# Lymphatus/caesium-clt

Hardware: NVIDIA H100
Metric: megapixels/sec JPEG q=80 4K re-encode (higher is better)
Workload: dtype i32

## Files before the change

caesium-clt_b200/csrc/jpeg_gpuenc.cu:

```cuda
#include <cuda_runtime.h>
#include <cub/device/device_scan.cuh>
#include <cuda_pipeline.h>
#include <algorithm>
#include <chrono>
#include <cstring>
#include "jpeg_gpuenc.h"
#include "stream_wait.h"
#include "launch_timer.h"

namespace b200 {

using namespace ge;

__global__ void k_ge_groups(const Scan *__restrict__ scans, const uint32_t *__restrict__ meta, const int *__restrict__ evkey,
                            const int *__restrict__ prev, const uint32_t *__restrict__ tsum, uint32_t *__restrict__ gcount, uint32_t *__restrict__ hist)
{
    __shared__ uint32_t eob[16];
    const Scan s = scans[blockIdx.y];
    if (s.mode != MODE_AC_FIRST && s.mode != MODE_AC_REFINE) return;
    if ((int)(blockIdx.x * blockDim.x) > s.nblocks) return;
    if (threadIdx.x < 16) eob[threadIdx.x] = 0;
    __syncthreads();
    const int b = blockIdx.x * blockDim.x + threadIdx.x;
    if (b <= s.nblocks && (b == s.nblocks || meta_event(meta[s.unit_base + b]))) {
        int pg;
        if (b < s.nblocks) pg = prev[s.unit_base + b];
        else { const long long last = s.unit_base + s.nblocks - 1; pg = max(prev[last], evkey[last]); }
        const int pl = pg >= s.unit_base ? (int)(pg - s.unit_base) : -1;
        assign_groups(meta + s.unit_base, tsum + s.unit_base, s.nblocks, pl, b, gcount + s.unit_base,
                      [&](uint32_t c) { atomicAdd(&eob[eob_symbol(c) >> 4], 1u); });
    }
    __syncthreads();
    if (threadIdx.x < 16 && eob[threadIdx.x]) atomicAdd(&hist[((size_t)s.tab_base + 2 + s.tbl[0]) * 256 + (threadIdx.x << 4)], eob[threadIdx.x]);
}

__global__ void k_ge_tables(const uint32_t *__restrict__ hist, Table *__restrict__ tabs, DhtOut *__restrict__ dht)
{
    __shared__ long long freq[257];
    __shared__ int codesize[257], others[257];
    __shared__ uint8_t bits[33];
    const int t = blockIdx.x, lane = threadIdx.x;
    const uint32_t *f = hist + (size_t)t * 256;
    for (int i = lane; i < 257; i += 32) { freq[i] = i < 256 ? (long long)f[i] : 1; codesize[i] = 0; others[i] = -1; }
    if (lane == 0) for (int i = 0; i < 33; i++) bits[i] = 0;
    __syncwarp();
    auto warp_argmin = [&](int exclude) {
        unsigned long long v = 1000000000ULL; int c = -1;
        for (int i = lane; i < 257; i += 32) { const unsigned long long fi = (unsigned long long)freq[i]; if (fi && fi <= v && i != exclude) { v = fi; c = i; } }
        const unsigned hi = (unsigned)(v >> 32), lo = (unsigned)v;
        const unsigned mhi = __reduce_min_sync(0xFFFFFFFFu, hi);
        const unsigned mlo = __reduce_min_sync(0xFFFFFFFFu, hi == mhi ? lo : 0xFFFFFFFFu);
        return __reduce_max_sync(0xFFFFFFFFu, (hi == mhi && lo == mlo) ? c : -1);
    };
    for (;;) {
        const int c1 = warp_argmin(-1);
        const int c2 = c1 < 0 ? -1 : warp_argmin(c1);
        if (c2 < 0) break;
        if (lane == 0) {
            int a = c1, b = c2;
            freq[a] += freq[b]; freq[b] = 0;
            codesize[a]++; while (others[a] >= 0) { a = others[a]; codesize[a]++; }
            others[a] = b;
            codesize[b]++; while (others[b] >= 0) { b = others[b]; codesize[b]++; }
        }
        __syncwarp();
    }
    if (lane == 0) {
        Table &T = tabs[t];
        for (int i = 0; i <= 256; i++) if (codesize[i]) bits[codesize[i] > 32 ? 32 : codesize[i]]++;
        for (int i = 32; i > 16; i--) while (bits[i] > 0) {
            int j = i - 2; while (bits[j] == 0) j--;
            bits[i] -= 2; bits[i - 1]++; bits[j + 1] += 2; bits[j]--;
        }
        int i = 16; while (i > 0 && bits[i] == 0) i--;
        if (i > 0) bits[i]--;
        int start[34];
        for (int l = 0; l < 34; l++) start[l] = 0;
        for (int s = 0; s <= 255; s++) if (codesize[s]) start[min(codesize[s], 32) + 1]++;
        for (int l = 1; l < 34; l++) start[l] += start[l - 1];
        const int p = start[33];
        for (int s = 0; s <= 255; s++) if (codesize[s]) T.vals[start[min(codesize[s], 32)]++] = (uint8_t)s;
        T.nvals = p;
        for (int k = 0; k < 17; k++) T.bits[k] = bits[k];
        for (int s = 0; s < 256; s++) T.code_len[s] = 0;
        uint32_t code = 0; int k = 0;
        for (int l = 1; l <= 16; l++) { for (int n = 0; n < bits[l]; n++, k++) T.code_len[T.vals[k]] = (code++ << 8) | (uint32_t)l; code <<= 1; }
        DhtOut &D = dht[t];
        D.nvals = p;
        for (int k2 = 0; k2 < 17; k2++) D.bits[k2] = bits[k2];
        for (int k2 = 0; k2 < p; k2++) D.vals[k2] = T.vals[k2];
    }
}

__global__ void k_ge_scanout(const Scan *__restrict__ scans, int nscans, const uint32_t *__restrict__ bitlen, const uint32_t *__restrict__ bitoff, uint32_t *__restrict__ total,
                             ScanOut *__restrict__ so, uint32_t words_cap, uint32_t groups_cap, uint32_t *__restrict__ flags)
{
    const int lane = threadIdx.x;
    uint32_t wbase = 0, gbase = 0;
    for (int c0 = 0; c0 < nscans; c0 += 32) {
        const int i = c0 + lane;
        uint32_t tb = 0;
        if (i < nscans) { const Scan s = scans[i]; const long long last = s.unit_base + s.nblocks - 1; tb = s.nblocks ? bitoff[last] + bitlen[last] - bitoff[s.unit_base] : 0; }
        const uint32_t nbytes = (tb + 7) / 8, ng = (nbytes + 15) / 16, nw = i < nscans ? (tb + 31) / 32 + 1 : 0;
        uint32_t wi = nw, gi = i < nscans ? ng : 0;
        for (int d = 1; d < 32; d <<= 1) { const uint32_t a = __shfl_up_sync(0xFFFFFFFFu, wi, d), b = __shfl_up_sync(0xFFFFFFFFu, gi, d); if (lane >= d) { wi += a; gi += b; } }
        if (i < nscans) { total[i] = tb; ScanOut o; o.total_bits = tb; o.nbytes = nbytes; o.ngroups = ng; o.group_base = gbase + gi - ng; o.word_base = wbase + wi - nw; o.pad_ = 0; so[i] = o; }
        wbase += __shfl_sync(0xFFFFFFFFu, wi, 31); gbase += __shfl_sync(0xFFFFFFFFu, gi, 31);
    }
    __syncwarp();
    const bool ovf = wbase > words_cap || gbase > groups_cap;
    if (lane == 0) { flags[0] = ovf ? 1u : 0u; flags[1] = wbase; flags[2] = gbase; flags[3] = 0; flags[4] = 0; }
    if (ovf) for (int i = lane; i < nscans; i += 32) { so[i].total_bits = 0; so[i].nbytes = 0; so[i].ngroups = 0; so[i].group_base = 0; so[i].word_base = 0; }
}

__global__ void k_ge_zero(const ScanOut *__restrict__ so, uint32_t *__restrict__ words)
{
    const ScanOut o = so[blockIdx.y];
    if (!o.total_bits) return;
    const uint32_t n = (o.total_bits + 31) / 32 + 1;
    uint32_t *w = words + o.word_base;
    for (uint32_t i = blockIdx.x * blockDim.x + threadIdx.x; i < n; i += gridDim.x * blockDim.x) w[i] = 0;
}

constexpr int ENC_THREADS = 128;
constexpr int TILE_PITCH = 72;
typedef int16_t Tile[ENC_THREADS][TILE_PITCH];

__device__ __forceinline__ void stage_tile(Tile &tile, const BlockComp &bc, int i0, int nblk)
{
    const uint4 *src = reinterpret_cast<const uint4 *>(bc.coef + bc.comp_off + (long long)i0 * 64);
    const int n = min(ENC_THREADS, nblk - i0) * 8;
#pragma unroll
    for (int k = 0; k < 8; k++) { const int q = threadIdx.x + k * ENC_THREADS; if (q < n) __pipeline_memcpy_async(&tile[q >> 3][(q & 7) * 8], src + q, 16); }
    __pipeline_commit();
}
__device__ __forceinline__ void wait_tile()
{
    __pipeline_wait_prior(0);
    __syncthreads();
}

__device__ __forceinline__ void stage_visits(EncVisit *vis, const BlockComp &bc)
{
    if ((int)threadIdx.x < bc.nscan) vis[threadIdx.x] = bc.visit[threadIdx.x];
}
__device__ __forceinline__ BlockRef ref_of(const EncVisit &v, const BlockComp &bc, const Tile &tile, int i0, int row, int col)
{
    BlockRef r;
    r.blk = tile[threadIdx.x]; r.prev = nullptr; r.slot = 0;
    if (v.mode == MODE_SEQ || v.mode == MODE_DC_FIRST) {
        const int p = enc_dc_prev(bc, v.ns, row, col);
        if (p >= i0 && p < i0 + ENC_THREADS) r.prev = tile[p - i0];
        else if (p >= 0) r.prev = bc.coef + bc.comp_off + (long long)p * 64;
    }
    return r;
}

template <class T>
__device__ __forceinline__ KindTabs<T> kind_tabs(T *tab, const EncVisit &v) { return KindTabs<T>{tab + ENC_DC_ENTRY, tab + v.ac_entry}; }

__device__ __forceinline__ Masks3 load_masks(const Masks3 *__restrict__ masks, const BlockComp &bc, int i)
{
    const unsigned long long *q = reinterpret_cast<const unsigned long long *>(masks + bc.mask_base + i);
    Masks3 M;
    M.m[0] = __ldg(q); M.m[1] = __ldg(q + 1); M.m[2] = __ldg(q + 2);
    return M;
}

struct SmemHist {
    KindTabs<uint32_t> h;
    __device__ void sym(int kind, int, int symbol, int, unsigned) { atomicAdd((kind ? h.ac : h.dc) + symbol, 1u); }
    __device__ void raw64(int, unsigned long long) {}
};
__global__ void __launch_bounds__(ENC_THREADS) k_geb_classify(const BlockComp *__restrict__ comps, uint32_t *__restrict__ meta, int *__restrict__ evkey,
                                                              uint32_t *__restrict__ tail, Masks3 *__restrict__ masks, uint32_t *__restrict__ hist)
{
    __shared__ __align__(16) Tile tile;
    __shared__ uint32_t h[ENC_TAB_ENTRIES];
    __shared__ EncVisit vis[ENC_MAX_VISITS];
    const BlockComp &bc = comps[blockIdx.y];
    const int nblk = bc.bw * bc.bh, i0 = blockIdx.x * ENC_THREADS, i = i0 + threadIdx.x;
    if (i0 >= nblk) return;
    stage_tile(tile, bc, i0, nblk);
    for (int k = threadIdx.x; k < ENC_TAB_ENTRIES; k += ENC_THREADS) h[k] = 0;
    stage_visits(vis, bc);
    wait_tile();
    if (i < nblk) {
        const int row = i / bc.bw, col = i - row * bc.bw;
        const Masks3 M = make_masks3(tile[threadIdx.x]);
        masks[bc.mask_base + i] = M;
        for (int j = 0; j < bc.nscan; j++) {
            const EncVisit &v = vis[j];
            const int u = enc_unit_of(bc, v.ns, row, col);
            if (u < 0) continue;
            const uint32_t m = classify_m(v, M);
            const int g = v.unit_base + u;
            meta[g] = m; evkey[g] = meta_event(m) ? g : -1; tail[g] = (uint32_t)meta_tail(m);
            SmemHist sk{kind_tabs(h, v)};
            gen_block_m(v, v.tbl, ref_of(v, bc, tile, i0, row, col), M, 0, sk);
        }
    }
    __syncthreads();
    for (int k = threadIdx.x; k < ENC_TAB_ENTRIES; k += ENC_THREADS) {
        int symbol; const int t = enc_entry_table(bc, k, symbol);
        if (h[k]) atomicAdd(&hist[(size_t)t * 256 + symbol], h[k]);
    }
}

__global__ void __launch_bounds__(ENC_THREADS) k_geb_len(const BlockComp *__restrict__ comps, const uint32_t *__restrict__ gcount, const Table *__restrict__ tabs,
                                                         uint32_t *__restrict__ bitlen, const Masks3 *__restrict__ masks)
{
    __shared__ __align__(16) Tile tile;
    __shared__ uint8_t tl[ENC_TAB_ENTRIES];
    __shared__ EncVisit vis[ENC_MAX_VISITS];
    const BlockComp &bc = comps[blockIdx.y];
    const int nblk = bc.bw * bc.bh, i0 = blockIdx.x * ENC_THREADS, i = i0 + threadIdx.x;
    if (i0 >= nblk) return;
    stage_tile(tile, bc, i0, nblk);
    const Masks3 M = load_masks(masks, bc, min(i, nblk - 1));
    stage_visits(vis, bc);
    for (int k = threadIdx.x; k < ENC_TAB_ENTRIES; k += ENC_THREADS) {
        int symbol; const int t = enc_entry_table(bc, k, symbol);
        if (t >= 0) tl[k] = (uint8_t)tabs[t].code_len[symbol];
    }
    wait_tile();
    if (i >= nblk) return;
    const int row = i / bc.bw, col = i - row * bc.bw;
    for (int j = 0; j < bc.nscan; j++) {
        const EncVisit &v = vis[j];
        const int u = enc_unit_of(bc, v.ns, row, col);
        if (u < 0) continue;
        LenSinkT<KindTabs<const uint8_t>> sk{kind_tabs<const uint8_t>(tl, v)};
        gen_block_m(v, v.tbl, ref_of(v, bc, tile, i0, row, col), M, gcount[v.unit_base + u], sk);
        bitlen[v.unit_base + u] = (uint32_t)sk.bits;
    }
}

__global__ void __launch_bounds__(ENC_THREADS) k_geb_emit(const BlockComp *__restrict__ comps, const uint32_t *__restrict__ gcount, const Table *__restrict__ tabs,
                                                          const uint32_t *__restrict__ bitoff, uint32_t *__restrict__ words, const Masks3 *__restrict__ masks, const ScanOut *__restrict__ so,
                                                          const uint32_t *__restrict__ flags)
{
    __shared__ __align__(16) Tile tile;
    __shared__ uint32_t tc[ENC_TAB_ENTRIES];
    __shared__ EncVisit vis[ENC_MAX_VISITS];
    __shared__ uint32_t vword[ENC_MAX_VISITS], vbit0[ENC_MAX_VISITS];
    if (flags[0]) return;
    const BlockComp &bc = comps[blockIdx.y];
    const int nblk = bc.bw * bc.bh, i0 = blockIdx.x * ENC_THREADS, i = i0 + threadIdx.x;
    if (i0 >= nblk) return;
    stage_tile(tile, bc, i0, nblk);
    const Masks3 M = load_masks(masks, bc, min(i, nblk - 1));
    stage_visits(vis, bc);
    if ((int)threadIdx.x < bc.nscan) {
        const EncVisit &v = bc.visit[threadIdx.x];
        vword[threadIdx.x] = so[v.scan].word_base; vbit0[threadIdx.x] = bitoff[v.unit_base];
    }
    for (int k = threadIdx.x; k < ENC_TAB_ENTRIES; k += ENC_THREADS) {
        int symbol; const int t = enc_entry_table(bc, k, symbol);
        if (t >= 0) tc[k] = tabs[t].code_len[symbol];
    }
    wait_tile();
    if (i >= nblk) return;
    const int row = i / bc.bw, col = i - row * bc.bw;
    auto orw = [&](long long w, uint32_t v) { if (v) atomicOr(&words[w], v); };
    auto stw = [&](long long w, uint32_t v) { words[w] = v; };
    for (int j = 0; j < bc.nscan; j++) {
        const EncVisit &v = vis[j];
        const int u = enc_unit_of(bc, v.ns, row, col);
        if (u < 0) continue;
        EmitSink<decltype(orw), decltype(stw), KindTabs<const uint32_t>> sk(kind_tabs<const uint32_t>(tc, v), orw, stw, (long long)vword[j],
                                                                            (unsigned long long)(bitoff[v.unit_base + u] - vbit0[j]));
        gen_block_m(v, v.tbl, ref_of(v, bc, tile, i0, row, col), M, gcount[v.unit_base + u], sk);
        sk.finish();
    }
}

__device__ __forceinline__ uint32_t scan_byte(const uint32_t *__restrict__ w, uint32_t i, uint32_t nbytes, uint32_t total_bits)
{
    uint32_t b = (w[i >> 2] >> (24 - 8 * (i & 3))) & 0xFF;
    if (i == nbytes - 1 && (total_bits & 7)) b |= (1u << (8 - (total_bits & 7))) - 1u;
    return b;
}

__global__ void k_ge_ffcount(const ScanOut *__restrict__ so, int nscans, const uint32_t *__restrict__ words, uint32_t *__restrict__ ffcount, uint32_t groups_cap,
                             const uint32_t *__restrict__ flags)
{
    if ((int)blockIdx.y == nscans) {
        const uint32_t used = flags[0] ? 0u : flags[2];
        for (uint32_t g = used + blockIdx.x * blockDim.x + threadIdx.x; g < groups_cap; g += gridDim.x * blockDim.x) ffcount[g] = 0;
        return;
    }
    const ScanOut o = so[blockIdx.y];
    const uint32_t *w = words + o.word_base;
    for (uint32_t g = blockIdx.x * blockDim.x + threadIdx.x; g < o.ngroups; g += gridDim.x * blockDim.x) {
        uint32_t n = 0;
        for (uint32_t i = g * 16; i < g * 16 + 16 && i < o.nbytes; i++) n += scan_byte(w, i, o.nbytes, o.total_bits) == 0xFF;
        ffcount[o.group_base + g] = n;
    }
}

__global__ void k_ge_layout(const ScanOut *__restrict__ so, int scans_per_image, int nimages, const uint32_t *__restrict__ ffcount, const uint32_t *__restrict__ ffoff,
                            uint32_t *__restrict__ out_off, uint32_t *__restrict__ out_len, uint32_t out_image_stride, uint32_t *__restrict__ flags)
{
    const int im = blockIdx.x * blockDim.x + threadIdx.x;
    if (im >= nimages) return;
    uint32_t off = 0;
    for (int k = 0; k < scans_per_image; k++) {
        const int si = im * scans_per_image + k;
        const ScanOut o = so[si];
        uint32_t ff = 0;
        if (o.ngroups) { const uint32_t lastg = o.group_base + o.ngroups - 1; ff = ffoff[lastg] + ffcount[lastg] - ffoff[o.group_base]; }
        out_off[si] = off; out_len[si] = o.nbytes + ff;
        off += o.nbytes + ff;
    }
    atomicMax(&flags[3], off);
    if (off > out_image_stride) atomicOr(&flags[4], 1u);
}

__global__ void k_ge_scatter(const ScanOut *__restrict__ so, const uint32_t *__restrict__ words, const uint32_t *__restrict__ ffoff,
                             const uint32_t *__restrict__ out_off, uint8_t *__restrict__ out, int scans_per_image, size_t out_image_stride, const uint32_t *__restrict__ flags)
{
    if (flags[4]) return;
    const ScanOut o = so[blockIdx.y];
    const uint32_t *w = words + o.word_base;
    uint8_t *base = out + (size_t)(blockIdx.y / scans_per_image) * out_image_stride + out_off[blockIdx.y];
    for (uint32_t g = blockIdx.x * blockDim.x + threadIdx.x; g < o.ngroups; g += gridDim.x * blockDim.x) {
        uint8_t *dst = base + (size_t)g * 16 + (ffoff[o.group_base + g] - ffoff[o.group_base]);
        for (uint32_t i = g * 16; i < g * 16 + 16 && i < o.nbytes; i++) {
            const uint32_t b = scan_byte(w, i, o.nbytes, o.total_bits);
            *dst++ = (uint8_t)b;
            if (b == 0xFF) *dst++ = 0;
        }
    }
}

__global__ void k_ge_fill_dummy(int16_t *__restrict__ coef, long long comp_off, int bw, int bh, int rbw, int rbh, int hs)
{
    const int i = blockIdx.x * blockDim.x + threadIdx.x;
    if (i >= bw * bh) return;
    const int row = i / bw, col = i - row * bw;
    if (row < rbh && col < rbw) return;
    int r = row, c = col;
    while (r >= rbh || c >= rbw) { if (r >= rbh) { c = (c / hs) * hs + hs - 1; r--; } else c = rbw - 1; }
    int16_t *base = coef + comp_off;
    int16_t *dst = base + ((long long)row * bw + col) * 64;
    const int16_t dc = base[((long long)r * bw + c) * 64];
    for (int k = 1; k < 64; k++) dst[k] = 0;
    dst[0] = dc;
}

static inline size_t align_up(size_t v, size_t a) { return (v + a - 1) / a * a; }
static inline int cdiv(long long a, long long b) { return (int)((a + b - 1) / b); }

GpuEncoder::~GpuEncoder()
{
    if (ev_sizes) cudaEventDestroy((cudaEvent_t)ev_sizes);
}

bool GpuEncoder::size_back_buffers(size_t image_bytes, std::string &err)
{
    const int NS = (int)plan.scans.size();
    if (nimg != cap_nimg) { cap_nimg = nimg; est_image_bytes = 0; }
    if (image_bytes <= est_image_bytes && words_cap) return true;
    est_image_bytes = image_bytes + image_bytes / 8;
    image_bytes = est_image_bytes;
    words_cap = (uint32_t)std::min<size_t>((size_t)nimg * (image_bytes / 4 + 1) + 2 * (size_t)NS + 64, 0xFFFFFF00u);
    groups_cap = (uint32_t)((size_t)words_cap / 4 + NS + 1);
    out_stride = align_up(image_bytes + image_bytes / 8 + 1024, 256);
    auto grow = [&](auto &buf, size_t need) { return buf.reserve(need, Grow::Pow2Half, err, &generation); };
    if (!grow(d_words, (size_t)words_cap * 4 + 64) || !grow(d_ffcount, (size_t)groups_cap * 4 + 4) || !grow(d_ffoff, (size_t)groups_cap * 4 + 4) ||
        !grow(d_out, out_stride * nimg)) return false;
    size_t tb3 = 0; cub::DeviceScan::ExclusiveSum((void *)nullptr, tb3, d_ffcount.get(), d_ffoff.get(), (int)groups_cap, (cudaStream_t)0);
    return grow(d_temp, tb3 + 256);
}

bool GpuEncoder::prepare(const JpegGeom &g, bool progressive, int16_t *const *d_coefs, int nimages, void *stream_, size_t out_bytes_hint, std::string &err)
{
    cudaStream_t st = (cudaStream_t)stream_;
    geom = g; prog = progressive;
    std::vector<const int16_t *> bases(d_coefs, d_coefs + nimages);
    coef_bases.assign(d_coefs, d_coefs + nimages);
    gpuenc_plan(g, progressive, bases.data(), nimages, plan);
    nimg = nimages;
    const int NS = (int)plan.scans.size();
    const long long U = plan.total_units;
    if (U >= (1ll << 31)) { err = "batch too large for the entropy encoder"; return false; }
    overflow = false;
    for (auto &sc_ : plan.scans) if (!masks_cover(sc_.mode, sc_.Al)) { err = "scan script outside the device encoder's mask range"; overflow = true; return false; }
    if (!plan.on_chip) { err = "scan script outside the device encoder's on-chip table slots"; overflow = true; return false; }
    if (!ev_sizes) { cudaEvent_t e; CU(cudaEventCreateWithFlags(&e, cudaEventDisableTiming | (stream_wait_mode() == 0 ? 0 : cudaEventBlockingSync))); ev_sizes = e; }
    auto grow = [&](auto &buf, size_t need) { return buf.reserve(need, Grow::Pow2Half, err, &generation); };
    const int NC = (int)plan.comps.size();
    if (!grow(d_scans, NS * sizeof(Scan)) || !grow(d_comps, NC * sizeof(BlockComp)) ||
        !grow(d_meta, U * 4) || !grow(d_evkey, U * 4) || !grow(d_prev, U * 4) || !grow(d_tail, U * 4) || !grow(d_tsum, U * 4) ||
        !grow(d_gcount, U * 4) || !grow(d_bitlen, U * 4) || !grow(d_bitoff, U * 4) ||
        !grow(d_hist, (size_t)NS * 4 * 256 * 4) || !grow(d_tabs, (size_t)NS * 4 * sizeof(Table)) || !grow(d_dht, (size_t)NS * 4 * sizeof(DhtOut)) ||
        !grow(d_total, (size_t)NS * 4) || !grow(d_so, (size_t)NS * sizeof(ScanOut)) || !grow(d_outoff, (size_t)NS * 4) || !grow(d_outlen, (size_t)NS * 4) ||
        !grow(d_flags, 64) || !grow(d_masks, (size_t)plan.total_comp_blocks * sizeof(Masks3))) return false;
    o_scans = 0; o_total = o_scans + align_up((size_t)NS * sizeof(Scan), 256); o_outlen = o_total + align_up((size_t)NS * 4, 256);
    o_dht = o_outlen + align_up((size_t)NS * 4, 256); o_comps = o_dht + align_up((size_t)NS * 4 * sizeof(DhtOut), 256);
    o_flags = o_comps + align_up((size_t)NC * sizeof(BlockComp), 256);
    const size_t small_bytes = o_flags + 256;
    if (!grow(h_small, small_bytes)) return false;
    size_t tb1 = 0, tb2 = 0;
    cub::DeviceScan::ExclusiveScan((void *)nullptr, tb1, d_evkey.get(), d_prev.get(), cub::Max(), -1, (int)U, st);
    cub::DeviceScan::ExclusiveSum((void *)nullptr, tb2, d_tail.get(), d_tsum.get(), (int)U, st);
    if (!grow(d_temp, std::max(tb1, tb2) + 256)) return false;
    const size_t coef_bytes = (size_t)g.total_coefs * 2;
    if (coef_bytes != learned_for) { learned_for = coef_bytes; learned_image_bytes = 0; }
    size_t est = out_bytes_hint ? out_bytes_hint / nimages + out_bytes_hint / nimages / 4 : coef_bytes / 3;
    est = std::max(est, learned_image_bytes + learned_image_bytes / 8) + 8192;
    est = std::min(est, coef_bytes * 2 + (size_t)plan.scans_per_image * 64 + 8192);
    if (!size_back_buffers(est, err)) return false;
    memcpy(h_small + o_scans, plan.scans.data(), NS * sizeof(Scan));
    memcpy(h_small + o_comps, plan.comps.data(), NC * sizeof(BlockComp));
    (void)st;
    return true;
}

bool GpuEncoder::upload(void *stream_, std::string &err)
{
    cudaStream_t st = (cudaStream_t)stream_;
    const int NS = (int)plan.scans.size(), NC = (int)plan.comps.size();
    CU(cudaMemcpyAsync(d_scans, h_small + o_scans, NS * sizeof(Scan), cudaMemcpyHostToDevice, st));
    CU(cudaMemcpyAsync(d_comps, h_small + o_comps, NC * sizeof(BlockComp), cudaMemcpyHostToDevice, st));
    return true;
}

unsigned long long GpuEncoder::signature() const
{
    unsigned long long h = 1469598103934665603ull;
    auto mix = [&](unsigned long long v) { h = (h ^ v) * 1099511628211ull; };
    mix((unsigned long long)nimg); mix((unsigned long long)plan.scans.size()); mix((unsigned long long)plan.comps.size()); mix((unsigned long long)plan.total_units);
    mix((unsigned long long)plan.max_comp_blocks); mix((unsigned long long)plan.scans_per_image); mix(words_cap); mix(groups_cap); mix(out_stride); mix(generation);
    mix((unsigned long long)geom.width); mix((unsigned long long)geom.height); mix(prog ? 1 : 0);
    for (int c = 0; c < geom.ncomp; c++) { mix((unsigned long long)geom.bw[c]); mix((unsigned long long)geom.bh[c]); mix((unsigned long long)geom.rbw[c]); mix((unsigned long long)geom.rbh[c]); mix((unsigned long long)geom.hs[c]); }
    for (auto pb : coef_bases) mix((unsigned long long)(uintptr_t)pb);
    int max_units = 0; for (auto &sc : plan.scans) max_units = std::max(max_units, sc.nblocks);
    mix((unsigned long long)max_units);
    return h;
}

bool GpuEncoder::enqueue_sizes(void *stream_, std::string &err)
{
    cudaStream_t st = (cudaStream_t)stream_;
    const int NS = (int)plan.scans.size();
    uint32_t *h_total = reinterpret_cast<uint32_t *>(h_small + o_total), *h_flags = reinterpret_cast<uint32_t *>(h_small + o_flags);
    k_ge_scanout<<<1, 32, 0, st>>>(d_scans, NS, d_bitlen, d_bitoff, d_total, d_so, words_cap, groups_cap, d_flags);
    LT_MARK("k_ge_scanout");
    CU(cudaMemcpyAsync(h_total, d_total, (size_t)NS * 4, cudaMemcpyDeviceToHost, st));
    CU(cudaMemcpyAsync(h_flags, d_flags, 12, cudaMemcpyDeviceToHost, st));
    LT_MARK("copy");
    return true;
}
bool GpuEncoder::mark_sizes(void *stream_, std::string &err)
{
    CU(cudaEventRecord((cudaEvent_t)ev_sizes, (cudaStream_t)stream_));
    return true;
}

bool GpuEncoder::enqueue_back(void *stream_, std::string &err)
{
    cudaStream_t st = (cudaStream_t)stream_;
    const int NS = (int)plan.scans.size(), NC = (int)plan.comps.size();
    uint32_t *h_flags = reinterpret_cast<uint32_t *>(h_small + o_flags);
    const dim3 gb(cdiv(plan.max_comp_blocks, ENC_THREADS), NC);
    k_ge_zero<<<dim3(64, NS), 256, 0, st>>>(d_so, d_words);
    LT_MARK("k_ge_zero");
    k_geb_emit<<<gb, ENC_THREADS, 0, st>>>(d_comps, d_gcount, d_tabs, d_bitoff, d_words, d_masks, d_so, d_flags);
    LT_MARK("k_geb_emit");
    k_ge_ffcount<<<dim3(32, NS + 1), 128, 0, st>>>(d_so, NS, d_words, d_ffcount, groups_cap, d_flags);
    LT_MARK("k_ge_ffcount");
    size_t tb = d_temp.capacity();
    cub::DeviceScan::ExclusiveSum(d_temp, tb, d_ffcount.get(), d_ffoff.get(), (int)groups_cap, st);
    LT_MARK("cub_scan");
    k_ge_layout<<<cdiv(nimg, 64), 64, 0, st>>>(d_so, plan.scans_per_image, nimg, d_ffcount, d_ffoff, d_outoff, d_outlen, (uint32_t)out_stride, d_flags);
    LT_MARK("k_ge_layout");
    k_ge_scatter<<<dim3(32, NS), 128, 0, st>>>(d_so, d_words, d_ffoff, d_outoff, d_out, plan.scans_per_image, out_stride, d_flags);
    LT_MARK("k_ge_scatter");
    CU(cudaMemcpyAsync(h_small + o_outlen, d_outlen, (size_t)NS * 4, cudaMemcpyDeviceToHost, st));
    CU(cudaMemcpyAsync(h_small + o_dht, d_dht, (size_t)NS * 4 * sizeof(DhtOut), cudaMemcpyDeviceToHost, st));
    CU(cudaMemcpyAsync(h_flags + 4, d_flags, 32, cudaMemcpyDeviceToHost, st));
    CU(cudaGetLastError());
    launches += 7;
    return true;
}

bool GpuEncoder::enqueue(void *stream_, bool fill_dummy, std::string &err)
{
    return enqueue_front(stream_, fill_dummy, err) && enqueue_sizes(stream_, err) && mark_sizes(stream_, err) && enqueue_back(stream_, err);
}

bool GpuEncoder::enqueue_front(void *stream_, bool fill_dummy, std::string &err)
{
    cudaStream_t st = (cudaStream_t)stream_;
    const JpegGeom &g = geom;
    const int NS = (int)plan.scans.size(), NC = (int)plan.comps.size();
    const long long U = plan.total_units;
    int max_units = 0; for (auto &s : plan.scans) max_units = std::max(max_units, s.nblocks);
    launches = 0;
    const dim3 gb(cdiv(plan.max_comp_blocks, ENC_THREADS), NC);
    if (fill_dummy) {
        for (int im = 0; im < nimg; im++) for (int cc = 0; cc < g.ncomp; cc++) {
            if (g.rbw[cc] == g.bw[cc] && g.rbh[cc] == g.bh[cc]) continue;
            k_ge_fill_dummy<<<cdiv((long long)g.bw[cc] * g.bh[cc], 256), 256, 0, st>>>(coef_bases[im], g.comp_offset[cc], g.bw[cc], g.bh[cc], g.rbw[cc], g.rbh[cc], g.hs[cc]);
            LT_MARK("k_ge_fill_dummy");
            launches++;
        }
    }
    const dim3 gu1(cdiv(max_units + 1, 128), NS);
    CU(cudaMemsetAsync(d_hist, 0, (size_t)NS * 4 * 256 * 4, st));
    LT_MARK("memset");
    k_geb_classify<<<gb, ENC_THREADS, 0, st>>>(d_comps, d_meta, d_evkey, d_tail, d_masks, d_hist);
    LT_MARK("k_geb_classify");
    size_t tb = d_temp.capacity();
    cub::DeviceScan::ExclusiveScan(d_temp, tb, d_evkey.get(), d_prev.get(), cub::Max(), -1, (int)U, st);
    LT_MARK("cub_scan");
    tb = d_temp.capacity();
    cub::DeviceScan::ExclusiveSum(d_temp, tb, d_tail.get(), d_tsum.get(), (int)U, st);
    LT_MARK("cub_scan");
    CU(cudaMemsetAsync(d_gcount, 0, U * 4, st));
    LT_MARK("memset");
    k_ge_groups<<<gu1, 128, 0, st>>>(d_scans, d_meta, d_evkey, d_prev, d_tsum, d_gcount, d_hist);
    LT_MARK("k_ge_groups");
    k_ge_tables<<<NS * 4, 32, 0, st>>>(d_hist, d_tabs, d_dht);
    LT_MARK("k_ge_tables");
    k_geb_len<<<gb, ENC_THREADS, 0, st>>>(d_comps, d_gcount, d_tabs, d_bitlen, d_masks);
    LT_MARK("k_geb_len");
    tb = d_temp.capacity();
    cub::DeviceScan::ExclusiveSum(d_temp, tb, d_bitlen.get(), d_bitoff.get(), (int)U, st);
    LT_MARK("cub_scan");
    launches += 7;
    CU(cudaGetLastError());
    return true;
}

bool GpuEncoder::finish(void *stream_, bool fetch, std::string &err)
{
    cudaStream_t st = (cudaStream_t)stream_;
    const int NS = (int)plan.scans.size(), spi = plan.scans_per_image;
    uint32_t *h_total = reinterpret_cast<uint32_t *>(h_small + o_total), *h_flags = reinterpret_cast<uint32_t *>(h_small + o_flags);
    uint32_t *h_outlen = reinterpret_cast<uint32_t *>(h_small + o_outlen);
    const DhtOut *h_dht = reinterpret_cast<const DhtOut *>(h_small + o_dht);
    for (int attempt = 0;; attempt++) {
        const auto tw0 = std::chrono::steady_clock::now();
        if (fetch) { CU(event_wait((cudaEvent_t)ev_sizes)); } else { CU(stream_wait(st)); }
        wait_sizes_ms = std::chrono::duration<double, std::milli>(std::chrono::steady_clock::now() - tw0).count();
        size_t img_max = 0, img = 0;
        for (int si = 0; si < NS; si++) { img += (h_total[si] + 7) / 8; if ((si + 1) % spi == 0) { img_max = std::max(img_max, img); img = 0; } }
        if (h_flags[0]) {
            if (attempt >= 3) { err = "entropy encoder could not size its buffers"; return false; }
            CU(stream_wait(st));
            if (!size_back_buffers(img_max + img_max / 16 + 4096, err)) return false;
            retries++;
            if (!enqueue_sizes(st, err) || !mark_sizes(st, err) || !enqueue_back(st, err)) return false;
            continue;
        }
        if (fetch) {
            copy_bytes = std::min(out_stride, align_up(img_max + img_max / 8 + 256, 256));
            if (!h_out.reserve(copy_bytes * nimg, Grow::Pow2Half, err, &generation)) return false;
            for (int im = 0; im < nimg; im++) CU(cudaMemcpyAsync(h_out + (size_t)im * copy_bytes, d_out + (size_t)im * out_stride, copy_bytes, cudaMemcpyDeviceToHost, st));
            CU(cudaGetLastError());
            const auto tw1 = std::chrono::steady_clock::now();
            CU(stream_wait(st));
            wait_final_ms = std::chrono::duration<double, std::milli>(std::chrono::steady_clock::now() - tw1).count();
        }
        if (h_flags[4 + 4]) {
            if (attempt >= 3) { err = "entropy encoder could not size its output"; return false; }
            if (!size_back_buffers((size_t)h_flags[4 + 3] + 4096, err)) return false;
            retries++;
            if (!enqueue_sizes(st, err) || !mark_sizes(st, err) || !enqueue_back(st, err)) return false;
            continue;
        }
        learned_image_bytes = std::max<size_t>(learned_image_bytes, h_flags[4 + 3]);
        if (fetch) {
            bool shortc = false;
            for (int im = 0; im < nimg && !shortc; im++) { size_t tot = 0; for (int k = 0; k < spi; k++) tot += h_outlen[im * spi + k]; shortc = tot > copy_bytes; }
            if (shortc) {
                if (!h_out.reserve(out_stride * nimg, Grow::Pow2Half, err, &generation)) return false;
                copy_bytes = out_stride;
                for (int j = 0; j < nimg; j++) CU(cudaMemcpyAsync(h_out + (size_t)j * copy_bytes, d_out + (size_t)j * out_stride, copy_bytes, cudaMemcpyDeviceToHost, st));
                CU(stream_wait(st));
            }
        }
        break;
    }
    results.assign((size_t)NS, EncodedScan());
    for (int si = 0; si < NS; si++) {
        EncodedScan &e = results[si];
        const int im = si / spi, k = si % spi;
        e.def = plan.defs[k];
        size_t off = 0; for (int j = 0; j < k; j++) off += h_outlen[im * spi + j];
        e.data = fetch ? h_out + (size_t)im * copy_bytes + off : nullptr; e.len = h_outlen[si];
        bool need[2][2]; jpeg_scan_tables_needed(geom, prog, e.def, need);
        for (int kind = 0; kind < 2; kind++) for (int t = 0; t < 2; t++) {
            e.has_tab[kind][t] = need[kind][t];
            const DhtOut &D = h_dht[(size_t)si * 4 + kind * 2 + t];
            memcpy(e.bits[kind][t], D.bits, 17); memcpy(e.vals[kind][t], D.vals, 256); e.nvals[kind][t] = D.nvals;
        }
    }
    return true;
}

bool GpuEncoder::encode(const JpegGeom &g, bool progressive, int16_t *const *d_coefs, int nimages, void *stream_, bool fill_dummy, std::string &err, size_t out_bytes_hint)
{
    return prepare(g, progressive, d_coefs, nimages, stream_, out_bytes_hint, err) && upload(stream_, err) && enqueue(stream_, fill_dummy, err) && finish(stream_, true, err);
}

}
```

caesium-clt_b200/csrc/jpeg_gpuenc.h:

```cpp
#pragma once
#include <cstdint>
#include <cstddef>
#include <string>
#include <vector>
#include "dev_buffer.h"
#include "jpeg_gpuenc_plan.h"

namespace b200 {

struct DhtOut { uint8_t bits[17]; uint8_t vals[256]; int32_t nvals; };
struct ScanOut { uint32_t total_bits, nbytes, ngroups, group_base, word_base, pad_; };

class GpuEncoder {
public:
    GpuEncoder() = default;
    ~GpuEncoder();
    GpuEncoder(const GpuEncoder &) = delete;
    GpuEncoder &operator=(const GpuEncoder &) = delete;
    bool encode(const JpegGeom &g, bool progressive, int16_t *const *d_coefs, int nimages, void *stream, bool fill_dummy, std::string &err, size_t out_bytes_hint = 0);
    bool prepare(const JpegGeom &g, bool progressive, int16_t *const *d_coefs, int nimages, void *stream, size_t out_bytes_hint, std::string &err);
    bool upload(void *stream, std::string &err);
    bool enqueue(void *stream, bool fill_dummy, std::string &err);
    bool enqueue_front(void *stream, bool fill_dummy, std::string &err);
    bool enqueue_sizes(void *stream, std::string &err);
    bool mark_sizes(void *stream, std::string &err);
    bool enqueue_back(void *stream, std::string &err);
    unsigned long long signature() const;
    bool finish(void *stream, bool fetch, std::string &err);
    int retries = 0;
    double wait_sizes_ms = 0, wait_final_ms = 0;
    std::vector<EncodedScan> results;
    GpuEncPlan plan;
    bool overflow = false;
    int launches = 0;
private:
    bool size_back_buffers(size_t image_bytes, std::string &err);
    unsigned long long generation = 0;
    int cap_nimg = 0;
    int nimg = 0;
    JpegGeom geom; bool prog = false;
    std::vector<int16_t *> coef_bases;
    void *ev_sizes = nullptr;
    uint32_t words_cap = 0, groups_cap = 0;
    size_t est_image_bytes = 0, learned_image_bytes = 0, learned_for = 0;
    DeviceBuffer<uint32_t> d_flags;
    size_t o_scans = 0, o_total = 0, o_outlen = 0, o_dht = 0, o_comps = 0, o_flags = 0;
    DeviceBuffer<ge::Scan> d_scans;
    DeviceBuffer<BlockComp> d_comps;
    DeviceBuffer<uint32_t> d_meta, d_tail, d_tsum, d_gcount, d_bitlen, d_bitoff;
    DeviceBuffer<int> d_evkey, d_prev;
    DeviceBuffer<uint32_t> d_hist;
    DeviceBuffer<ge::Table> d_tabs;
    DeviceBuffer<DhtOut> d_dht;
    DeviceBuffer<uint32_t> d_total;
    DeviceBuffer<ScanOut> d_so;
    DeviceBuffer<uint32_t> d_words;
    DeviceBuffer<ge::Masks3> d_masks;
    DeviceBuffer<uint32_t> d_ffcount, d_ffoff;
    DeviceBuffer<uint32_t> d_outoff, d_outlen;
    DeviceBuffer<uint8_t> d_out;
    DeviceBuffer<uint8_t> d_temp;
    PinnedBuffer<uint8_t> h_small;
    PinnedBuffer<uint8_t> h_out;
    size_t out_stride = 0, copy_bytes = 0;
};

}
```

caesium-clt_b200/csrc/jpeg_gpuenc_core.h:

```cpp
#pragma once
#include <cstdint>

#if defined(__CUDACC__)
#define GE_HD __host__ __device__ __forceinline__
#else
#define GE_HD inline
#endif

namespace b200 {
namespace ge {

enum ScanMode { MODE_SEQ = 0, MODE_DC_FIRST = 1, MODE_AC_FIRST = 2, MODE_AC_REFINE = 3 };

constexpr int EOBRUN_MAX = 0x7FFF;
constexpr int CORR_FLUSH = 1000 - 64 + 1;

struct Scan {
    const int16_t *coef;
    int mode, ns, Ss, Se, Al;
    int comp[3];
    int hs[3], vs[3], bw[3];
    long long comp_off[3];
    int tbl[3];
    int mcux, mcuy, blocks_per_mcu;
    int rbw, rbh;
    int nblocks;
    long long unit_base;
    int tab_base;
    long long word_base;
    long long word_cap;
};

struct Table {
    uint32_t code_len[256];
    uint8_t bits[17];
    uint8_t vals[256];
    int nvals;
};

GE_HD uint32_t meta_pack(bool event, bool contrib, int tail) { return (event ? 1u : 0u) | (contrib ? 2u : 0u) | ((uint32_t)tail << 8); }
GE_HD bool meta_event(uint32_t m) { return m & 1u; }
GE_HD bool meta_contrib(uint32_t m) { return m & 2u; }
GE_HD int meta_tail(uint32_t m) { return (int)(m >> 8); }

GE_HD int nbits_of(unsigned v)
{
#if defined(__CUDA_ARCH__)
    return 32 - __clz((int)v);
#else
    return v ? 32 - __builtin_clz(v) : 0;
#endif
}

struct BlockRef { const int16_t *blk; const int16_t *prev; int slot; };

GE_HD BlockRef locate(const Scan &s, int u)
{
    BlockRef r;
    if (s.ns == 1) {
        const int row = u / s.rbw, col = u - row * s.rbw;
        const int16_t *base = s.coef + s.comp_off[0];
        r.blk = base + ((long long)row * s.bw[0] + col) * 64;
        r.slot = 0;
        if (u == 0) r.prev = nullptr;
        else { const int pu = u - 1, prow = pu / s.rbw, pcol = pu - prow * s.rbw; r.prev = base + ((long long)prow * s.bw[0] + pcol) * 64; }
        return r;
    }
    const int m = u / s.blocks_per_mcu;
    int q = u - m * s.blocks_per_mcu, i = 0;
    while (q >= s.hs[i] * s.vs[i]) { q -= s.hs[i] * s.vs[i]; i++; }
    const int my = m / s.mcux, mx = m - my * s.mcux;
    const int by = q / s.hs[i], bx = q - by * s.hs[i];
    const int16_t *base = s.coef + s.comp_off[i];
    r.slot = i;
    r.blk = base + ((long long)(my * s.vs[i] + by) * s.bw[i] + mx * s.hs[i] + bx) * 64;
    if (q > 0) { const int pq = q - 1, pby = pq / s.hs[i], pbx = pq - pby * s.hs[i]; r.prev = base + ((long long)(my * s.vs[i] + pby) * s.bw[i] + mx * s.hs[i] + pbx) * 64; }
    else if (m == 0) r.prev = nullptr;
    else { const int pm = m - 1, pmy = pm / s.mcux, pmx = pm - pmy * s.mcux; r.prev = base + ((long long)(pmy * s.vs[i] + s.vs[i] - 1) * s.bw[i] + pmx * s.hs[i] + s.hs[i] - 1) * 64; }
    return r;
}

GE_HD int ctz64(unsigned long long m)
{
#if defined(__CUDA_ARCH__)
    return __ffsll((long long)m) - 1;
#else
    return __builtin_ctzll(m);
#endif
}
GE_HD int msb64(unsigned long long m)
{
#if defined(__CUDA_ARCH__)
    return 63 - __clzll((long long)m);
#else
    return m ? 63 - __builtin_clzll(m) : -1;
#endif
}
GE_HD int popc64(unsigned long long m)
{
#if defined(__CUDA_ARCH__)
    return __popcll(m);
#else
    return __builtin_popcountll(m);
#endif
}
GE_HD unsigned long long band_mask(int Ss, int Se) { return (Se >= 63 ? ~0ull : ((1ull << (Se + 1)) - 1ull)) & ~((1ull << Ss) - 1ull); }

struct Masks3 { unsigned long long m[3]; };
GE_HD bool masks_cover(int mode, int Al) { return mode == MODE_AC_REFINE ? Al <= 1 : Al <= 2; }
GE_HD unsigned long long mask_at(const Masks3 &M, int t) { return t == 0 ? M.m[0] : t == 1 ? M.m[1] : M.m[2]; }

GE_HD uint32_t interleave16(uint32_t acc)
{
    uint32_t x = acc & 0xFFFFu, y = acc >> 16;
    x = (x | (x << 8)) & 0x00FF00FFu; x = (x | (x << 4)) & 0x0F0F0F0Fu; x = (x | (x << 2)) & 0x33333333u; x = (x | (x << 1)) & 0x55555555u;
    y = (y | (y << 8)) & 0x00FF00FFu; y = (y | (y << 4)) & 0x0F0F0F0Fu; y = (y | (y << 2)) & 0x33333333u; y = (y | (y << 1)) & 0x55555555u;
    return x | (y << 1);
}
GE_HD void masks_word(uint32_t w, int jj , uint32_t (&acc)[3])
{
    const uint32_t sb = (w >> 15) & 0x00010001u;
    const uint32_t a = (w ^ (sb * 0xFFFFu)) + sb;
    const uint32_t pos = 0x00010001u << jj;
    acc[0] |= ((a + 0x7FFF7FFFu) >> (15 - jj)) & pos;
    acc[1] |= (((a & 0xFFFEFFFEu) + 0x7FFF7FFFu) >> (15 - jj)) & pos;
    acc[2] |= (((a & 0xFFFCFFFCu) + 0x7FFF7FFFu) >> (15 - jj)) & pos;
}
GE_HD Masks3 make_masks3(const int16_t *__restrict__ blk)
{
    Masks3 M;
    uint32_t lo[3] = {0, 0, 0}, hi[3] = {0, 0, 0};
#if defined(__CUDA_ARCH__)
    const uint4 *v = reinterpret_cast<const uint4 *>(blk);
#pragma unroll
    for (int j = 0; j < 8; j++) {
        const uint4 q = v[j];
        const uint32_t w[4] = {q.x, q.y, q.z, q.w};
#pragma unroll
        for (int i = 0; i < 4; i++) { if (j < 4) masks_word(w[i], (4 * j + i) & 15, lo); else masks_word(w[i], (4 * j + i) & 15, hi); }
    }
#else
    for (int j = 0; j < 32; j++) {
        const uint32_t w = (uint32_t)(uint16_t)blk[2 * j] | ((uint32_t)(uint16_t)blk[2 * j + 1] << 16);
        if (j < 16) masks_word(w, j, lo); else masks_word(w, j - 16, hi);
    }
#endif
    for (int t = 0; t < 3; t++) M.m[t] = ((unsigned long long)interleave16(hi[t]) << 32) | interleave16(lo[t]);
    return M;
}
inline Masks3 make_masks3_reference(const int16_t *blk)
{
    Masks3 M; M.m[0] = M.m[1] = M.m[2] = 0;
    for (int k = 0; k < 64; k++) { int a = blk[k]; if (a < 0) a = -a; for (int t = 0; t < 3; t++) if (a >= (1 << t)) M.m[t] |= 1ull << k; }
    return M;
}

template <class S>
GE_HD uint32_t classify_m(const S &s, const Masks3 &M)
{
    if (s.mode == MODE_SEQ || s.mode == MODE_DC_FIRST) return meta_pack(true, false, 0);
    const unsigned long long band = band_mask(s.Ss, s.Se);
    const unsigned long long mA = mask_at(M, s.Al) & band, mB = (s.mode == MODE_AC_REFINE ? mask_at(M, s.Al + 1) : 0ull) & band;
    if (s.mode == MODE_AC_FIRST) { const int last = msb64(mA); return meta_pack(last >= 0, last < s.Se, 0); }
    const int last_new = msb64(mA & ~mB);
    int tail;
    if (last_new < 0) tail = popc64(mB);
    else if (last_new >= 63) tail = 0;
    else tail = popc64(mB & ~((2ull << last_new) - 1ull));
    return meta_pack(last_new >= 0, last_new < s.Se, tail);
}
GE_HD uint32_t classify(const Scan &s, const int16_t *blk)
{
    if (s.mode == MODE_SEQ || s.mode == MODE_DC_FIRST) return meta_pack(true, false, 0);
    return classify_m(s, make_masks3(blk));
}

template <class Sink>
GE_HD void gen_dc(int value_shifted, int pred_shifted, int tbl, Sink &sk)
{
    int temp = value_shifted - pred_shifted, temp2 = temp;
    if (temp < 0) { temp = -temp; temp2--; }
    const int nb = nbits_of((unsigned)temp);
    sk.sym(0, tbl, nb, nb, (unsigned)temp2);
}

GE_HD int eob_symbol(unsigned count) { return (nbits_of(count) - 1) << 4; }
template <class Sink>
GE_HD void gen_eob_token(unsigned count, int tbl, Sink &sk)
{
    sk.sym(1, tbl, eob_symbol(count), nbits_of(count) - 1, count);
}

template <class S, class Sink>
GE_HD void gen_block_m(const S &s, int tbl, const BlockRef &b, const Masks3 &M, unsigned group_count, Sink &sk)
{
    const int16_t *blk = b.blk;
    if (s.mode == MODE_DC_FIRST) { gen_dc(blk[0] >> s.Al, b.prev ? (b.prev[0] >> s.Al) : 0, tbl, sk); return; }
    if (s.mode == MODE_SEQ) {
        gen_dc(blk[0], b.prev ? b.prev[0] : 0, tbl, sk);
        int prevk = 0;
        for (unsigned long long m = M.m[0] & ~1ull; m; m &= m - 1) {
            const int k = ctz64(m);
            int r = k - prevk - 1; prevk = k;
            while (r > 15) { sk.sym(1, tbl, 0xF0, 0, 0); r -= 16; }
            int t = blk[k], t2 = t; if (t < 0) { t = -t; t2--; }
            const int nb = nbits_of((unsigned)t);
            sk.sym(1, tbl, (r << 4) + nb, nb, (unsigned)t2);
        }
        if (prevk != 63) sk.sym(1, tbl, 0, 0, 0);
        return;
    }
    const unsigned long long band = band_mask(s.Ss, s.Se);
    const unsigned long long mA = mask_at(M, s.Al) & band;
    const unsigned long long mB = (s.mode == MODE_AC_REFINE ? mask_at(M, s.Al + 1) : 0ull) & band;
    if (s.mode == MODE_AC_FIRST) {
        int prevk = s.Ss - 1;
        for (unsigned long long m = mA; m; m &= m - 1) {
            const int k = ctz64(m);
            int r = k - prevk - 1; prevk = k;
            while (r > 15) { sk.sym(1, tbl, 0xF0, 0, 0); r -= 16; }
            int t = blk[k], t2;
            if (t < 0) { t = (-t) >> s.Al; t2 = ~t; } else { t >>= s.Al; t2 = t; }
            const int nb = nbits_of((unsigned)t);
            sk.sym(1, tbl, (r << 4) + nb, nb, (unsigned)t2);
        }
        if (group_count) gen_eob_token(group_count, tbl, sk);
        return;
    }
    const unsigned long long newm = mA & ~mB;
    const int last_new = msb64(newm);
    const int EOB = last_new < 0 ? 0 : last_new;
    int r = 0, prevk = s.Ss - 1;
    int npend = 0; unsigned long long pend64 = 0;
    for (unsigned long long m = mA; m; m &= m - 1) {
        const int k = ctz64(m);
        r += k - prevk - 1; prevk = k;
        while (r > 15 && k <= EOB) {
            sk.sym(1, tbl, 0xF0, 0, 0); r -= 16;
            if (npend) { sk.raw64(npend, pend64); npend = 0; pend64 = 0; }
        }
        int t = blk[k];
        const bool neg = t < 0;
        if (neg) t = -t;
        t >>= s.Al;
        if ((mB >> k) & 1ull) { pend64 = (pend64 << 1) | (unsigned)(t & 1); npend++; continue; }
        sk.sym(1, tbl, (r << 4) + 1, 1, neg ? 0u : 1u);
        if (npend) { sk.raw64(npend, pend64); npend = 0; pend64 = 0; }
        r = 0;
    }
    if (group_count) gen_eob_token(group_count, tbl, sk);
    if (npend) sk.raw64(npend, pend64);
}
template <class Sink>
GE_HD void gen_block(const Scan &s, const BlockRef &b, unsigned group_count, Sink &sk)
{
    if (s.mode == MODE_DC_FIRST) { Masks3 none; none.m[0] = none.m[1] = none.m[2] = 0; gen_block_m(s, s.tbl[b.slot], b, none, group_count, sk); return; }
    gen_block_m(s, s.tbl[b.slot], b, make_masks3(b.blk), group_count, sk);
}

struct ScanTabs {
    const Table *t = nullptr;
    ScanTabs() = default;
    GE_HD ScanTabs(const Table *p) : t(p) {}
    GE_HD uint32_t operator()(int kind, int tbl, int symbol) const { return t[kind * 2 + tbl].code_len[symbol]; }
};
template <class T>
struct KindTabs {
    T *dc, *ac;
    GE_HD uint32_t operator()(int kind, int, int symbol) const { return (kind ? ac : dc)[symbol]; }
};

template <class AddFn>
struct HistSink {
    AddFn add;
    GE_HD explicit HistSink(AddFn f) : add(f) {}
    GE_HD void sym(int kind, int tbl, int symbol, int, unsigned) { add((kind * 2 + tbl) * 256 + symbol); }
    GE_HD void raw64(int, unsigned long long) {}
};

template <class Tabs = ScanTabs>
struct LenSinkT {
    Tabs tabs;
    unsigned long long bits = 0;
    GE_HD void sym(int kind, int tbl, int symbol, int nb, unsigned) { bits += (tabs(kind, tbl, symbol) & 0xFFu) + nb; }
    GE_HD void raw64(int nb, unsigned long long) { bits += nb; }
};
using LenSink = LenSinkT<>;

GE_HD uint32_t shl_or_zero(uint32_t v, int s)
{
#if defined(__CUDA_ARCH__)
    return __funnelshift_lc(0u, v, (unsigned)s);
#else
    return s >= 32 ? 0u : v << s;
#endif
}

template <class OrFn, class StFn = OrFn, class Tabs = ScanTabs>
struct EmitSink {
    Tabs tabs;
    OrFn orw;
    StFn stw;
    long long wpos, first;
    uint32_t cur = 0; int n;
    GE_HD EmitSink(Tabs t, OrFn f, StFn g, long long word_base, unsigned long long bitoff)
        : tabs(t), orw(f), stw(g), wpos(word_base + (long long)(bitoff >> 5)), first(wpos), n((int)(bitoff & 31)) {}
    GE_HD EmitSink(Tabs t, OrFn f, long long word_base, unsigned long long bitoff) : EmitSink(t, f, f, word_base, bitoff) {}
    GE_HD void put(uint32_t code, int len)
    {
        if (!len) return;
        const int fill = n + len;
        if (fill < 32) { cur |= code << (32 - fill); n = fill; return; }
        const int r = fill - 32;
        const uint32_t w = cur | (code >> r);
        if (wpos == first) orw(wpos, w); else stw(wpos, w);
        wpos++;
        cur = shl_or_zero(code, 32 - r); n = r;
    }
    GE_HD void sym(int kind, int tbl, int symbol, int nb, unsigned extra)
    {
        const uint32_t e = tabs(kind, tbl, symbol);
        put(((e >> 8) << nb) | (extra & ((1u << nb) - 1u)), (int)(e & 0xFFu) + nb);
    }
    GE_HD void raw64(int nb, unsigned long long v)
    {
        if (nb > 32) { put((unsigned)(v >> 32), nb - 32); put((unsigned)v, 32); } else put((unsigned)v, nb);
    }
    GE_HD void finish() { if (n > 0) orw(wpos, cur); }
};

struct NoCount { GE_HD void operator()(uint32_t) const {} };
template <class CountFn = NoCount>
GE_HD void assign_groups(const uint32_t *meta, const uint32_t *tsum, int nblocks, int prev_ev, int b, uint32_t *gcount, CountFn &&counted = CountFn())
{
    auto group = [&](int j, uint32_t c) { gcount[j] = c; counted(c); };
    int gs = prev_ev < 0 ? 0 : (meta_contrib(meta[prev_ev]) ? prev_ev : prev_ev + 1);
    if (gs >= b) return;
    const int count = b - gs;
    const uint32_t tend = b < nblocks ? tsum[b] : tsum[nblocks - 1] + (uint32_t)meta_tail(meta[nblocks - 1]);
    const uint32_t tailbits = tend - tsum[gs];
    if (count < EOBRUN_MAX && tailbits <= (uint32_t)CORR_FLUSH) { group(gs, (uint32_t)count); return; }
    int start = gs, n = 0; unsigned be = 0;
    for (int j = gs; j < b; j++) {
        n++; be += (unsigned)meta_tail(meta[j]);
        if (n == EOBRUN_MAX || be > (unsigned)CORR_FLUSH) { group(start, (uint32_t)n); start = j + 1; n = 0; be = 0; }
    }
    if (n > 0) group(start, (uint32_t)n);
}

GE_HD void build_table(const uint32_t *freq_in, Table &t, int *codesize , int *others , long long *freq )
{
    uint8_t bits[33];
    for (int i = 0; i < 33; i++) bits[i] = 0;
    for (int i = 0; i < 256; i++) { freq[i] = freq_in[i]; codesize[i] = 0; others[i] = -1; }
    freq[256] = 1; codesize[256] = 0; others[256] = -1;
    for (;;) {
        int c1 = -1, c2 = -1; long long v = 1000000000LL;
        for (int i = 0; i <= 256; i++) if (freq[i] && freq[i] <= v) { v = freq[i]; c1 = i; }
        v = 1000000000LL;
        for (int i = 0; i <= 256; i++) if (freq[i] && freq[i] <= v && i != c1) { v = freq[i]; c2 = i; }
        if (c2 < 0) break;
        freq[c1] += freq[c2]; freq[c2] = 0;
        codesize[c1]++; while (others[c1] >= 0) { c1 = others[c1]; codesize[c1]++; }
        others[c1] = c2;
        codesize[c2]++; while (others[c2] >= 0) { c2 = others[c2]; codesize[c2]++; }
    }
    for (int i = 0; i <= 256; i++) if (codesize[i]) bits[codesize[i] > 32 ? 32 : codesize[i]]++;
    for (int i = 32; i > 16; i--) while (bits[i] > 0) {
        int j = i - 2; while (bits[j] == 0) j--;
        bits[i] -= 2; bits[i - 1]++; bits[j + 1] += 2; bits[j]--;
    }
    int i = 16; while (i > 0 && bits[i] == 0) i--;
    if (i > 0) bits[i]--;
    for (int k = 0; k < 17; k++) t.bits[k] = bits[k];
    int p = 0;
    for (int l = 1; l <= 32; l++) for (int s = 0; s <= 255; s++) if (codesize[s] == l) t.vals[p++] = (uint8_t)s;
    t.nvals = p;
    for (int s = 0; s < 256; s++) t.code_len[s] = 0;
    uint32_t code = 0; int k = 0;
    for (int l = 1; l <= 16; l++) { for (int n = 0; n < t.bits[l]; n++, k++) t.code_len[t.vals[k]] = (code++ << 8) | (uint32_t)l; code <<= 1; }
}

}
}
```

caesium-clt_b200/csrc/jpeg_gpuenc_plan.h:

```cpp
#pragma once
#include <algorithm>
#include <vector>
#include "jpeg_gpuenc_core.h"
#include "jpeg_host.h"

namespace b200 {

constexpr int ENC_MAX_VISITS = 6, ENC_AC_SLOTS = 3, ENC_DC_SLOTS = 1, ENC_DC_SYMBOLS = 17;
constexpr int ENC_TAB_ENTRIES = ENC_AC_SLOTS * 256 + ENC_DC_SLOTS * ENC_DC_SYMBOLS;
constexpr int ENC_DC_ENTRY = ENC_AC_SLOTS * 256;

struct EncVisit {
    int scan;
    int mode, Ss, Se, Al, ns;
    int tbl;
    int unit_base;
    int ac_entry;
};

struct BlockComp {
    const int16_t *coef;
    long long comp_off;
    int bw, bh, rbw, rbh, hs, vs;
    int q_base, blocks_per_mcu, mcux;
    int nscan;
    EncVisit visit[ENC_MAX_VISITS];
    int tab[ENC_AC_SLOTS + ENC_DC_SLOTS];
    long long mask_base;
};

GE_HD int enc_unit_of(const BlockComp &bc, int ns, int row, int col)
{
    if (ns == 1) return (row < bc.rbh && col < bc.rbw) ? row * bc.rbw + col : -1;
    const int m = (row / bc.vs) * bc.mcux + col / bc.hs, q = bc.q_base + (row % bc.vs) * bc.hs + (col % bc.hs);
    return m * bc.blocks_per_mcu + q;
}
GE_HD int enc_dc_prev(const BlockComp &bc, int ns, int row, int col)
{
    if (ns == 1) return col > 0 ? row * bc.bw + col - 1 : row > 0 ? (row - 1) * bc.bw + bc.rbw - 1 : -1;
    if (col % bc.hs) return row * bc.bw + col - 1;
    if (row % bc.vs) return (row - 1) * bc.bw + col + bc.hs - 1;
    if (col) return (row + bc.vs - 1) * bc.bw + col - 1;
    if (row) return (row - 1) * bc.bw + bc.mcux * bc.hs - 1;
    return -1;
}

GE_HD int enc_entry_table(const BlockComp &bc, int k, int &symbol)
{
    if (k < ENC_DC_ENTRY) { symbol = k & 255; return bc.tab[k >> 8]; }
    symbol = k - ENC_DC_ENTRY; return bc.tab[ENC_AC_SLOTS];
}

struct GpuEncPlan {
    std::vector<BlockComp> comps;
    bool on_chip = true;
    int max_comp_blocks = 0;
    std::vector<ge::Scan> scans;
    std::vector<ScanDef> defs;
    int scans_per_image = 0;
    long long units_per_image = 0, words_per_image = 0;
    long long total_units = 0, total_words = 0, total_comp_blocks = 0;
};

inline void gpuenc_plan(const JpegGeom &g, bool progressive, const int16_t *const *coef_base, int nimages, GpuEncPlan &p)
{
    ScanDef sc[16];
    const int ns = jpeg_scan_script(g, progressive, sc);
    p.defs.assign(sc, sc + ns);
    p.scans_per_image = ns;
    p.scans.clear();
    long long unit = 0, word = 0;
    for (int im = 0; im < nimages; im++) {
        for (int si = 0; si < ns; si++) {
            const ScanDef &d = sc[si];
            ge::Scan s{};
            s.coef = coef_base[im];
            s.ns = d.ns; s.Ss = d.Ss; s.Se = d.Se; s.Al = d.Al;
            if (!progressive) s.mode = ge::MODE_SEQ;
            else if (d.Ss == 0) s.mode = ge::MODE_DC_FIRST;
            else s.mode = d.Ah == 0 ? ge::MODE_AC_FIRST : ge::MODE_AC_REFINE;
            s.blocks_per_mcu = 0;
            for (int i = 0; i < d.ns; i++) {
                const int c = d.ci[i];
                s.comp[i] = c; s.hs[i] = g.hs[c]; s.vs[i] = g.vs[c]; s.bw[i] = g.bw[c]; s.comp_off[i] = g.comp_offset[c]; s.tbl[i] = c ? 1 : 0;
                s.blocks_per_mcu += g.hs[c] * g.vs[c];
            }
            s.mcux = g.mcux; s.mcuy = g.mcuy;
            s.rbw = g.rbw[d.ci[0]]; s.rbh = g.rbh[d.ci[0]];
            s.nblocks = d.ns > 1 ? g.mcux * g.mcuy * s.blocks_per_mcu : s.rbw * s.rbh;
            s.unit_base = unit; unit += s.nblocks;
            s.tab_base = (int)p.scans.size() * 4;
            s.word_base = word; s.word_cap = (long long)s.nblocks * 32 + 64; word += s.word_cap;
            p.scans.push_back(s);
        }
        if (im == 0) { p.units_per_image = unit; p.words_per_image = word; }
    }
    p.total_units = unit; p.total_words = word;
    p.comps.clear(); p.max_comp_blocks = 0; p.total_comp_blocks = 0; p.on_chip = true;
    for (int im = 0; im < nimages; im++) {
        int qb = 0;
        for (int c = 0; c < g.ncomp; c++) {
            BlockComp bc{};
            bc.coef = coef_base[im]; bc.comp_off = g.comp_offset[c];
            bc.bw = g.bw[c]; bc.bh = g.bh[c]; bc.rbw = g.rbw[c]; bc.rbh = g.rbh[c]; bc.hs = g.hs[c]; bc.vs = g.vs[c];
            bc.q_base = qb; bc.mcux = g.mcux;
            bc.blocks_per_mcu = 0; for (int cc = 0; cc < g.ncomp; cc++) bc.blocks_per_mcu += g.hs[cc] * g.vs[cc];
            qb += g.hs[c] * g.vs[c];
            bc.nscan = 0;
            int nac = 0, ndc = 0;
            for (int k = 0; k < ENC_AC_SLOTS + ENC_DC_SLOTS; k++) bc.tab[k] = -1;
            for (int si = 0; si < ns; si++) for (int i = 0; i < sc[si].ns; i++) {
                if (sc[si].ci[i] != c) continue;
                const ge::Scan &s = p.scans[(size_t)im * ns + si];
                const bool dc = s.mode == ge::MODE_SEQ || s.mode == ge::MODE_DC_FIRST, ac = s.mode != ge::MODE_DC_FIRST;
                if (bc.nscan == ENC_MAX_VISITS || nac + ac > ENC_AC_SLOTS || ndc + dc > ENC_DC_SLOTS) { p.on_chip = false; continue; }
                EncVisit &v = bc.visit[bc.nscan++];
                v.scan = im * ns + si; v.mode = s.mode; v.Ss = s.Ss; v.Se = s.Se; v.Al = s.Al; v.ns = s.ns; v.tbl = s.tbl[i];
                v.unit_base = (int)s.unit_base;
                v.ac_entry = ac ? nac * 256 : 0;
                if (ac) bc.tab[nac++] = s.tab_base + 2 + v.tbl;
                if (dc) bc.tab[ENC_AC_SLOTS + ndc++] = s.tab_base + v.tbl;
            }
            bc.mask_base = p.total_comp_blocks; p.total_comp_blocks += (long long)bc.bw * bc.bh;
            p.comps.push_back(bc);
            p.max_comp_blocks = std::max(p.max_comp_blocks, bc.bw * bc.bh);
        }
    }
}

}
```

Baseline: 40560.

## Compute scan sizes from histograms and emit single-component scans via per-CTA runs

Total bits per scan are now derived analytically from symbol histograms and code lengths, plus a correction count for refinement bits. This drops the per-block length pass and the prefix scan for single-component scans. Those scans are emitted into an arena as per-CTA contiguous runs, using a CTA-local exclusive sum and an atomic cursor, then relocated into the final bitstream by a placement kernel. The gain is fewer kernels and less per-block bitoff traffic. The cost is extra arena memory, a second copy pass, and more complex bookkeeping, and it relies on the analytic bit count being exact.

```diff
diff --git a/caesium-clt_b200/csrc/jpeg_gpuenc.cu b/caesium-clt_b200/csrc/jpeg_gpuenc.cu
--- a/caesium-clt_b200/csrc/jpeg_gpuenc.cu
+++ b/caesium-clt_b200/csrc/jpeg_gpuenc.cu
@@ -34,7 +34,7 @@
     if (threadIdx.x < 16 && eob[threadIdx.x]) atomicAdd(&hist[((size_t)s.tab_base + 2 + s.tbl[0]) * 256 + (threadIdx.x << 4)], eob[threadIdx.x]);
 }
 
-__global__ void k_ge_tables(const uint32_t *__restrict__ hist, Table *__restrict__ tabs, DhtOut *__restrict__ dht)
+__global__ void k_ge_tables(const uint32_t *__restrict__ hist, Table *__restrict__ tabs, DhtOut *__restrict__ dht, unsigned long long *__restrict__ tbits)
 {
     __shared__ long long freq[257];
     __shared__ int codesize[257], others[257];
@@ -90,39 +90,57 @@
         for (int k2 = 0; k2 < 17; k2++) D.bits[k2] = bits[k2];
         for (int k2 = 0; k2 < p; k2++) D.vals[k2] = T.vals[k2];
     }
-}
-
-__global__ void k_ge_scanout(const Scan *__restrict__ scans, int nscans, const uint32_t *__restrict__ bitlen, const uint32_t *__restrict__ bitoff, uint32_t *__restrict__ total,
-                             ScanOut *__restrict__ so, uint32_t words_cap, uint32_t groups_cap, uint32_t *__restrict__ flags)
+    __syncwarp();
+    const int kind = (t & 3) >> 1;
+    unsigned long long nb = 0;
+    for (int i = lane; i < 256; i += 32) if (f[i]) nb += (unsigned long long)f[i] * ((tabs[t].code_len[i] & 0xFFu) + (unsigned)sym_extra_bits(kind, i));
+    for (int d = 16; d; d >>= 1) nb += __shfl_xor_sync(0xFFFFFFFFu, nb, d);
+    if (lane == 0) tbits[t] = nb;
+}
+
+__global__ void k_ge_scanout(const Scan *__restrict__ scans, int nscans, const unsigned long long *__restrict__ tbits, const uint32_t *__restrict__ corr,
+                             uint32_t *__restrict__ total, ScanOut *__restrict__ so, uint32_t words_cap, uint32_t groups_cap, uint32_t *__restrict__ flags)
 {
     const int lane = threadIdx.x;
-    uint32_t wbase = 0, gbase = 0;
+    uint32_t wbase = 0, gbase = 0, abase = 0;
     for (int c0 = 0; c0 < nscans; c0 += 32) {
         const int i = c0 + lane;
-        uint32_t tb = 0;
-        if (i < nscans) { const Scan s = scans[i]; const long long last = s.unit_base + s.nblocks - 1; tb = s.nblocks ? bitoff[last] + bitlen[last] - bitoff[s.unit_base] : 0; }
+        uint32_t tb = 0, na = 0;
+        if (i < nscans) {
+            tb = (uint32_t)(tbits[4 * i] + tbits[4 * i + 1] + tbits[4 * i + 2] + tbits[4 * i + 3] + corr[i]);
+            na = scans[i].nruns ? (tb + 31) / 32 + scans[i].nruns : 0;
+        }
         const uint32_t nbytes = (tb + 7) / 8, ng = (nbytes + 15) / 16, nw = i < nscans ? (tb + 31) / 32 + 1 : 0;
-        uint32_t wi = nw, gi = i < nscans ? ng : 0;
-        for (int d = 1; d < 32; d <<= 1) { const uint32_t a = __shfl_up_sync(0xFFFFFFFFu, wi, d), b = __shfl_up_sync(0xFFFFFFFFu, gi, d); if (lane >= d) { wi += a; gi += b; } }
-        if (i < nscans) { total[i] = tb; ScanOut o; o.total_bits = tb; o.nbytes = nbytes; o.ngroups = ng; o.group_base = gbase + gi - ng; o.word_base = wbase + wi - nw; o.pad_ = 0; so[i] = o; }
-        wbase += __shfl_sync(0xFFFFFFFFu, wi, 31); gbase += __shfl_sync(0xFFFFFFFFu, gi, 31);
+        uint32_t wi = nw, gi = i < nscans ? ng : 0, ai = na;
+        for (int d = 1; d < 32; d <<= 1) {
+            const uint32_t a = __shfl_up_sync(0xFFFFFFFFu, wi, d), b = __shfl_up_sync(0xFFFFFFFFu, gi, d), c = __shfl_up_sync(0xFFFFFFFFu, ai, d);
+            if (lane >= d) { wi += a; gi += b; ai += c; }
+        }
+        if (i < nscans) {
+            total[i] = tb;
+            ScanOut o; o.total_bits = tb; o.nbytes = nbytes; o.ngroups = ng; o.group_base = gbase + gi - ng; o.word_base = wbase + wi - nw; o.arena_base = abase + ai - na;
+            so[i] = o;
+        }
+        wbase += __shfl_sync(0xFFFFFFFFu, wi, 31); gbase += __shfl_sync(0xFFFFFFFFu, gi, 31); abase += __shfl_sync(0xFFFFFFFFu, ai, 31);
     }
     __syncwarp();
     const bool ovf = wbase > words_cap || gbase > groups_cap;
     if (lane == 0) { flags[0] = ovf ? 1u : 0u; flags[1] = wbase; flags[2] = gbase; flags[3] = 0; flags[4] = 0; }
-    if (ovf) for (int i = lane; i < nscans; i += 32) { so[i].total_bits = 0; so[i].nbytes = 0; so[i].ngroups = 0; so[i].group_base = 0; so[i].word_base = 0; }
-}
-
-__global__ void k_ge_zero(const ScanOut *__restrict__ so, uint32_t *__restrict__ words)
+    if (ovf) for (int i = lane; i < nscans; i += 32) { so[i].total_bits = 0; so[i].nbytes = 0; so[i].ngroups = 0; so[i].group_base = 0; so[i].word_base = 0; so[i].arena_base = 0; }
+}
+
+__global__ void k_ge_zero(const Scan *__restrict__ scans, const ScanOut *__restrict__ so, uint32_t *__restrict__ words, uint32_t *__restrict__ arena)
 {
     const ScanOut o = so[blockIdx.y];
     if (!o.total_bits) return;
-    const uint32_t n = (o.total_bits + 31) / 32 + 1;
-    uint32_t *w = words + o.word_base;
-    for (uint32_t i = blockIdx.x * blockDim.x + threadIdx.x; i < n; i += gridDim.x * blockDim.x) w[i] = 0;
-}
-
-constexpr int ENC_THREADS = 128;
+    const uint32_t n = (o.total_bits + 31) / 32 + 1, nruns = (uint32_t)scans[blockIdx.y].nruns, na = nruns ? n - 1 + nruns : 0;
+    uint32_t *w = words + o.word_base, *a = arena + o.arena_base;
+    for (uint32_t i = blockIdx.x * blockDim.x + threadIdx.x; i < max(n, na); i += gridDim.x * blockDim.x) {
+        if (i < n) w[i] = 0;
+        if (i < na) a[i] = 0;
+    }
+}
+
 constexpr int TILE_PITCH = 72;
 typedef int16_t Tile[ENC_THREADS][TILE_PITCH];
 
@@ -173,16 +191,18 @@
     __device__ void raw64(int, unsigned long long) {}
 };
 __global__ void __launch_bounds__(ENC_THREADS) k_geb_classify(const BlockComp *__restrict__ comps, uint32_t *__restrict__ meta, int *__restrict__ evkey,
-                                                              uint32_t *__restrict__ tail, Masks3 *__restrict__ masks, uint32_t *__restrict__ hist)
+                                                              uint32_t *__restrict__ tail, Masks3 *__restrict__ masks, uint32_t *__restrict__ hist, uint32_t *__restrict__ corr)
 {
     __shared__ __align__(16) Tile tile;
     __shared__ uint32_t h[ENC_TAB_ENTRIES];
     __shared__ EncVisit vis[ENC_MAX_VISITS];
+    __shared__ uint32_t vcorr[ENC_MAX_VISITS];
     const BlockComp &bc = comps[blockIdx.y];
     const int nblk = bc.bw * bc.bh, i0 = blockIdx.x * ENC_THREADS, i = i0 + threadIdx.x;
     if (i0 >= nblk) return;
     stage_tile(tile, bc, i0, nblk);
     for (int k = threadIdx.x; k < ENC_TAB_ENTRIES; k += ENC_THREADS) h[k] = 0;
+    if (threadIdx.x < ENC_MAX_VISITS) vcorr[threadIdx.x] = 0;
     stage_visits(vis, bc);
     wait_tile();
     if (i < nblk) {
@@ -198,9 +218,12 @@
             meta[g] = m; evkey[g] = meta_event(m) ? g : -1; tail[g] = (uint32_t)meta_tail(m);
             SmemHist sk{kind_tabs(h, v)};
             gen_block_m(v, v.tbl, ref_of(v, bc, tile, i0, row, col), M, 0, sk);
+            const int nc = corr_bits_m(v, M);
+            if (nc) atomicAdd(&vcorr[j], (uint32_t)nc);
         }
     }
     __syncthreads();
+    if ((int)threadIdx.x < bc.nscan && vcorr[threadIdx.x]) atomicAdd(&corr[vis[threadIdx.x].scan], vcorr[threadIdx.x]);
     for (int k = threadIdx.x; k < ENC_TAB_ENTRIES; k += ENC_THREADS) {
         int symbol; const int t = enc_entry_table(bc, k, symbol);
         if (h[k]) atomicAdd(&hist[(size_t)t * 256 + symbol], h[k]);
@@ -228,51 +251,132 @@
     const int row = i / bc.bw, col = i - row * bc.bw;
     for (int j = 0; j < bc.nscan; j++) {
         const EncVisit &v = vis[j];
+        if (v.ns == 1) continue;
         const int u = enc_unit_of(bc, v.ns, row, col);
         if (u < 0) continue;
         LenSinkT<KindTabs<const uint8_t>> sk{kind_tabs<const uint8_t>(tl, v)};
         gen_block_m(v, v.tbl, ref_of(v, bc, tile, i0, row, col), M, gcount[v.unit_base + u], sk);
-        bitlen[v.unit_base + u] = (uint32_t)sk.bits;
-    }
-}
-
+        bitlen[v.lu_base + u] = (uint32_t)sk.bits;
+    }
+}
+constexpr int LEN_DC_THREADS = 256;
+__global__ void __launch_bounds__(LEN_DC_THREADS) k_geb_len_dc(const BlockComp *__restrict__ comps, const Table *__restrict__ tabs, uint32_t *__restrict__ bitlen)
+{
+    const BlockComp &bc = comps[blockIdx.y];
+    const int nblk = bc.bw * bc.bh, i = blockIdx.x * LEN_DC_THREADS + threadIdx.x;
+    if (i >= nblk) return;
+    const int row = i / bc.bw, col = i - row * bc.bw;
+    const int16_t *cb = bc.coef + bc.comp_off;
+    const Masks3 none{};
+    for (int j = 0; j < bc.nscan; j++) {
+        const EncVisit v = bc.visit[j];
+        if (v.ns == 1) continue;
+        const int p = enc_dc_prev(bc, v.ns, row, col);
+        const BlockRef r{cb + (long long)i * 64, p >= 0 ? cb + (long long)p * 64 : nullptr, 0};
+        LenSinkT<KindTabs<const uint32_t>> sk{KindTabs<const uint32_t>{tabs[bc.tab[ENC_AC_SLOTS]].code_len, nullptr}};
+        gen_block_m(v, v.tbl, r, none, 0, sk);
+        bitlen[v.lu_base + enc_unit_of(bc, v.ns, row, col)] = (uint32_t)sk.bits;
+    }
+}
+
+__device__ __forceinline__ uint32_t cta_exclusive_sum(uint32_t x, uint32_t *wsum , uint32_t &total)
+{
+    const int lane = threadIdx.x & 31, w = threadIdx.x >> 5;
+    uint32_t inc = x;
+    for (int d = 1; d < 32; d <<= 1) { const uint32_t y = __shfl_up_sync(0xFFFFFFFFu, inc, d); if (lane >= d) inc += y; }
+    if (lane == 31) wsum[w] = inc;
+    __syncthreads();
+    uint32_t base = 0, tot = 0;
+#pragma unroll
+    for (int k = 0; k < ENC_THREADS / 32; k++) { const uint32_t sk = wsum[k]; if (k < w) base += sk; tot += sk; }
+    total = tot;
+    return base + inc - x;
+}
+
+constexpr int ENC_SLOT_WORDS = 8;
 __global__ void __launch_bounds__(ENC_THREADS) k_geb_emit(const BlockComp *__restrict__ comps, const uint32_t *__restrict__ gcount, const Table *__restrict__ tabs,
                                                           const uint32_t *__restrict__ bitoff, uint32_t *__restrict__ words, const Masks3 *__restrict__ masks, const ScanOut *__restrict__ so,
-                                                          const uint32_t *__restrict__ flags)
+                                                          const uint32_t *__restrict__ flags, uint32_t *__restrict__ arena, uint32_t *__restrict__ cursor,
+                                                          uint32_t *__restrict__ runlen, uint32_t *__restrict__ runpos)
 {
     __shared__ __align__(16) Tile tile;
     __shared__ uint32_t tc[ENC_TAB_ENTRIES];
     __shared__ EncVisit vis[ENC_MAX_VISITS];
     __shared__ uint32_t vword[ENC_MAX_VISITS], vbit0[ENC_MAX_VISITS];
+    __shared__ uint32_t slot[ENC_SLOT_WORDS][ENC_THREADS];
+    __shared__ uint32_t wsum[ENC_THREADS / 32], run_word;
     if (flags[0]) return;
     const BlockComp &bc = comps[blockIdx.y];
     const int nblk = bc.bw * bc.bh, i0 = blockIdx.x * ENC_THREADS, i = i0 + threadIdx.x;
     if (i0 >= nblk) return;
+    const bool live = i < nblk;
     stage_tile(tile, bc, i0, nblk);
     const Masks3 M = load_masks(masks, bc, min(i, nblk - 1));
     stage_visits(vis, bc);
     if ((int)threadIdx.x < bc.nscan) {
         const EncVisit &v = bc.visit[threadIdx.x];
-        vword[threadIdx.x] = so[v.scan].word_base; vbit0[threadIdx.x] = bitoff[v.unit_base];
+        const ScanOut &o = so[v.scan];
+        vword[threadIdx.x] = v.ns > 1 ? o.word_base : o.arena_base; vbit0[threadIdx.x] = v.ns > 1 ? bitoff[v.lu_base] : 0;
     }
     for (int k = threadIdx.x; k < ENC_TAB_ENTRIES; k += ENC_THREADS) {
         int symbol; const int t = enc_entry_table(bc, k, symbol);
         if (t >= 0) tc[k] = tabs[t].code_len[symbol];
     }
     wait_tile();
-    if (i >= nblk) return;
     const int row = i / bc.bw, col = i - row * bc.bw;
     auto orw = [&](long long w, uint32_t v) { if (v) atomicOr(&words[w], v); };
     auto stw = [&](long long w, uint32_t v) { words[w] = v; };
+    auto ora = [&](long long w, uint32_t v) { if (v) atomicOr(&arena[w], v); };
+    auto sta = [&](long long w, uint32_t v) { arena[w] = v; };
+    auto sls = [&](long long w, uint32_t v) { if (w < ENC_SLOT_WORDS) slot[w][threadIdx.x] = v; };
+    typedef KindTabs<const uint32_t> KT;
     for (int j = 0; j < bc.nscan; j++) {
         const EncVisit &v = vis[j];
-        const int u = enc_unit_of(bc, v.ns, row, col);
-        if (u < 0) continue;
-        EmitSink<decltype(orw), decltype(stw), KindTabs<const uint32_t>> sk(kind_tabs<const uint32_t>(tc, v), orw, stw, (long long)vword[j],
-                                                                            (unsigned long long)(bitoff[v.unit_base + u] - vbit0[j]));
-        gen_block_m(v, v.tbl, ref_of(v, bc, tile, i0, row, col), M, gcount[v.unit_base + u], sk);
-        sk.finish();
-    }
+        const int u = live ? enc_unit_of(bc, v.ns, row, col) : -1;
+        if (v.ns > 1) {
+            if (u < 0) continue;
+            EmitSink<decltype(orw), decltype(stw), KT> sk(kind_tabs<const uint32_t>(tc, v), orw, stw, (long long)vword[j], (unsigned long long)(bitoff[v.lu_base + u] - vbit0[j]));
+            gen_block_m(v, v.tbl, ref_of(v, bc, tile, i0, row, col), M, gcount[v.unit_base + u], sk);
+            sk.finish();
+            continue;
+        }
+        uint32_t nb = 0;
+        if (u >= 0) {
+            EmitSink<decltype(sls), decltype(sls), KT> sk(kind_tabs<const uint32_t>(tc, v), sls, sls, 0, 0);
+            gen_block_m(v, v.tbl, ref_of(v, bc, tile, i0, row, col), M, gcount[v.unit_base + u], sk);
+            sk.finish();
+            nb = (uint32_t)sk.bits_written(0);
+        }
+        uint32_t L;
+        const uint32_t off = cta_exclusive_sum(nb, wsum, L);
+        if (threadIdx.x == 0) {
+            const uint32_t a = vword[j] + atomicAdd(&cursor[v.scan], (L + 31) / 32);
+            run_word = a; runlen[v.run_base + blockIdx.x] = L; runpos[v.run_base + blockIdx.x] = a;
+        }
+        __syncthreads();
+        const unsigned long long at = (unsigned long long)run_word * 32 + off;
+        if (nb <= ENC_SLOT_WORDS * 32) place_bits([&](long long k) { return slot[k][threadIdx.x]; }, nb, at, ora, sta);
+        else {
+            EmitSink<decltype(ora), decltype(sta), KT> sk(kind_tabs<const uint32_t>(tc, v), ora, sta, 0, at);
+            gen_block_m(v, v.tbl, ref_of(v, bc, tile, i0, row, col), M, gcount[v.unit_base + u], sk);
+            sk.finish();
+        }
+    }
+}
+
+constexpr int PLACE_THREADS = 128;
+__global__ void __launch_bounds__(PLACE_THREADS) k_ge_place(const Scan *__restrict__ scans, const ScanOut *__restrict__ so, const uint32_t *__restrict__ runlen,
+                                                            const uint32_t *__restrict__ runoff, const uint32_t *__restrict__ runpos, const uint32_t *__restrict__ arena,
+                                                            uint32_t *__restrict__ words, const uint32_t *__restrict__ flags)
+{
+    if (flags[0]) return;
+    const int nruns = scans[blockIdx.y].nruns, x = blockIdx.x * (PLACE_THREADS / 32) + (threadIdx.x >> 5);
+    if (x >= nruns) return;
+    const int r0 = scans[blockIdx.y].run_base, r = r0 + x;
+    const uint32_t *src = arena + runpos[r];
+    uint32_t *dst = words + so[blockIdx.y].word_base;
+    place_bits([&](long long k) { return src[k]; }, runlen[r], runoff[r] - runoff[r0],
+               [&](long long w, uint32_t v) { atomicOr(&dst[w], v); }, [&](long long w, uint32_t v) { dst[w] = v; }, threadIdx.x & 31, 32);
 }
 
 __device__ __forceinline__ uint32_t scan_byte(const uint32_t *__restrict__ w, uint32_t i, uint32_t nbytes, uint32_t total_bits)
@@ -360,15 +464,16 @@
 bool GpuEncoder::size_back_buffers(size_t image_bytes, std::string &err)
 {
     const int NS = (int)plan.scans.size();
+    auto grow = [&](auto &buf, size_t need) { return buf.reserve(need, Grow::Pow2Half, err, &generation); };
+    auto grow_arena = [&]() { return grow(d_arena, ((size_t)words_cap + (size_t)plan.total_runs) * 4 + 64); };
     if (nimg != cap_nimg) { cap_nimg = nimg; est_image_bytes = 0; }
-    if (image_bytes <= est_image_bytes && words_cap) return true;
+    if (image_bytes <= est_image_bytes && words_cap) return grow_arena();
     est_image_bytes = image_bytes + image_bytes / 8;
     image_bytes = est_image_bytes;
     words_cap = (uint32_t)std::min<size_t>((size_t)nimg * (image_bytes / 4 + 1) + 2 * (size_t)NS + 64, 0xFFFFFF00u);
     groups_cap = (uint32_t)((size_t)words_cap / 4 + NS + 1);
     out_stride = align_up(image_bytes + image_bytes / 8 + 1024, 256);
-    auto grow = [&](auto &buf, size_t need) { return buf.reserve(need, Grow::Pow2Half, err, &generation); };
-    if (!grow(d_words, (size_t)words_cap * 4 + 64) || !grow(d_ffcount, (size_t)groups_cap * 4 + 4) || !grow(d_ffoff, (size_t)groups_cap * 4 + 4) ||
+    if (!grow_arena() || !grow(d_words, (size_t)words_cap * 4 + 64) || !grow(d_ffcount, (size_t)groups_cap * 4 + 4) || !grow(d_ffoff, (size_t)groups_cap * 4 + 4) ||
         !grow(d_out, out_stride * nimg)) return false;
     size_t tb3 = 0; cub::DeviceScan::ExclusiveSum((void *)nullptr, tb3, d_ffcount.get(), d_ffoff.get(), (int)groups_cap, (cudaStream_t)0);
     return grow(d_temp, tb3 + 256);
@@ -383,7 +488,8 @@
     gpuenc_plan(g, progressive, bases.data(), nimages, plan);
     nimg = nimages;
     const int NS = (int)plan.scans.size();
-    const long long U = plan.total_units;
+    const long long U = plan.total_units, LU = std::max(plan.total_lunits, 1ll);
+    const int R = std::max(plan.total_runs, 1);
     if (U >= (1ll << 31)) { err = "batch too large for the entropy encoder"; return false; }
     overflow = false;
     for (auto &sc_ : plan.scans) if (!masks_cover(sc_.mode, sc_.Al)) { err = "scan script outside the device encoder's mask range"; overflow = true; return false; }
@@ -393,7 +499,8 @@
     const int NC = (int)plan.comps.size();
     if (!grow(d_scans, NS * sizeof(Scan)) || !grow(d_comps, NC * sizeof(BlockComp)) ||
         !grow(d_meta, U * 4) || !grow(d_evkey, U * 4) || !grow(d_prev, U * 4) || !grow(d_tail, U * 4) || !grow(d_tsum, U * 4) ||
-        !grow(d_gcount, U * 4) || !grow(d_bitlen, U * 4) || !grow(d_bitoff, U * 4) ||
+        !grow(d_gcount, U * 4) || !grow(d_bitlen, LU * 4) || !grow(d_bitoff, LU * 4) || !grow(d_corr, (size_t)NS * 4) || !grow(d_tbits, (size_t)NS * 4 * 8) ||
+        !grow(d_cursor, (size_t)NS * 4) || !grow(d_runlen, (size_t)R * 4) || !grow(d_runoff, (size_t)R * 4) || !grow(d_runpos, (size_t)R * 4) ||
         !grow(d_hist, (size_t)NS * 4 * 256 * 4) || !grow(d_tabs, (size_t)NS * 4 * sizeof(Table)) || !grow(d_dht, (size_t)NS * 4 * sizeof(DhtOut)) ||
         !grow(d_total, (size_t)NS * 4) || !grow(d_so, (size_t)NS * sizeof(ScanOut)) || !grow(d_outoff, (size_t)NS * 4) || !grow(d_outlen, (size_t)NS * 4) ||
         !grow(d_flags, 64) || !grow(d_masks, (size_t)plan.total_comp_blocks * sizeof(Masks3))) return false;
@@ -402,10 +509,12 @@
     o_flags = o_comps + align_up((size_t)NC * sizeof(BlockComp), 256);
     const size_t small_bytes = o_flags + 256;
     if (!grow(h_small, small_bytes)) return false;
-    size_t tb1 = 0, tb2 = 0;
+    size_t tb1 = 0, tb2 = 0, tb3 = 0, tb4 = 0;
     cub::DeviceScan::ExclusiveScan((void *)nullptr, tb1, d_evkey.get(), d_prev.get(), cub::Max(), -1, (int)U, st);
     cub::DeviceScan::ExclusiveSum((void *)nullptr, tb2, d_tail.get(), d_tsum.get(), (int)U, st);
-    if (!grow(d_temp, std::max(tb1, tb2) + 256)) return false;
+    cub::DeviceScan::ExclusiveSum((void *)nullptr, tb3, d_bitlen.get(), d_bitoff.get(), (int)LU, st);
+    cub::DeviceScan::ExclusiveSum((void *)nullptr, tb4, d_runlen.get(), d_runoff.get(), R, st);
+    if (!grow(d_temp, std::max(std::max(tb1, tb2), std::max(tb3, tb4)) + 256)) return false;
     const size_t coef_bytes = (size_t)g.total_coefs * 2;
     if (coef_bytes != learned_for) { learned_for = coef_bytes; learned_image_bytes = 0; }
     size_t est = out_bytes_hint ? out_bytes_hint / nimages + out_bytes_hint / nimages / 4 : coef_bytes / 3;
@@ -438,6 +547,7 @@
     for (auto pb : coef_bases) mix((unsigned long long)(uintptr_t)pb);
     int max_units = 0; for (auto &sc : plan.scans) max_units = std::max(max_units, sc.nblocks);
     mix((unsigned long long)max_units);
+    mix((unsigned long long)plan.total_lunits); mix((unsigned long long)plan.total_runs); mix((unsigned long long)plan.max_runs);
     return h;
 }
 
@@ -446,7 +556,7 @@
     cudaStream_t st = (cudaStream_t)stream_;
     const int NS = (int)plan.scans.size();
     uint32_t *h_total = reinterpret_cast<uint32_t *>(h_small + o_total), *h_flags = reinterpret_cast<uint32_t *>(h_small + o_flags);
-    k_ge_scanout<<<1, 32, 0, st>>>(d_scans, NS, d_bitlen, d_bitoff, d_total, d_so, words_cap, groups_cap, d_flags);
+    k_ge_scanout<<<1, 32, 0, st>>>(d_scans, NS, d_tbits, d_corr, d_total, d_so, words_cap, groups_cap, d_flags);
     LT_MARK("k_ge_scanout");
     CU(cudaMemcpyAsync(h_total, d_total, (size_t)NS * 4, cudaMemcpyDeviceToHost, st));
     CU(cudaMemcpyAsync(h_flags, d_flags, 12, cudaMemcpyDeviceToHost, st));
@@ -465,10 +575,36 @@
     const int NS = (int)plan.scans.size(), NC = (int)plan.comps.size();
     uint32_t *h_flags = reinterpret_cast<uint32_t *>(h_small + o_flags);
     const dim3 gb(cdiv(plan.max_comp_blocks, ENC_THREADS), NC);
-    k_ge_zero<<<dim3(64, NS), 256, 0, st>>>(d_so, d_words);
+    int n = 6;
+    if (plan.total_lunits) {
+        bool dc_only = true;
+        for (auto &sc : plan.scans) if (sc.ns > 1 && sc.mode != MODE_DC_FIRST) dc_only = false;
+        if (dc_only) {
+            k_geb_len_dc<<<dim3(cdiv(plan.max_comp_blocks, LEN_DC_THREADS), NC), LEN_DC_THREADS, 0, st>>>(d_comps, d_tabs, d_bitlen);
+            LT_MARK("k_geb_len_dc");
+        } else {
+            k_geb_len<<<gb, ENC_THREADS, 0, st>>>(d_comps, d_gcount, d_tabs, d_bitlen, d_masks);
+            LT_MARK("k_geb_len");
+        }
+        size_t tb = d_temp.capacity();
+        cub::DeviceScan::ExclusiveSum(d_temp, tb, d_bitlen.get(), d_bitoff.get(), (int)plan.total_lunits, st);
+        LT_MARK("cub_scan");
+        n += 2;
+    }
+    CU(cudaMemsetAsync(d_cursor, 0, (size_t)NS * 4, st));
+    LT_MARK("memset");
+    k_ge_zero<<<dim3(64, NS), 256, 0, st>>>(d_scans, d_so, d_words, d_arena);
     LT_MARK("k_ge_zero");
-    k_geb_emit<<<gb, ENC_THREADS, 0, st>>>(d_comps, d_gcount, d_tabs, d_bitoff, d_words, d_masks, d_so, d_flags);
+    k_geb_emit<<<gb, ENC_THREADS, 0, st>>>(d_comps, d_gcount, d_tabs, d_bitoff, d_words, d_masks, d_so, d_flags, d_arena, d_cursor, d_runlen, d_runpos);
     LT_MARK("k_geb_emit");
+    if (plan.total_runs) {
+        size_t tb = d_temp.capacity();
+        cub::DeviceScan::ExclusiveSum(d_temp, tb, d_runlen.get(), d_runoff.get(), plan.total_runs, st);
+        LT_MARK("cub_scan");
+        k_ge_place<<<dim3(cdiv(plan.max_runs, PLACE_THREADS / 32), NS), PLACE_THREADS, 0, st>>>(d_scans, d_so, d_runlen, d_runoff, d_runpos, d_arena, d_words, d_flags);
+        LT_MARK("k_ge_place");
+        n += 2;
+    }
     k_ge_ffcount<<<dim3(32, NS + 1), 128, 0, st>>>(d_so, NS, d_words, d_ffcount, groups_cap, d_flags);
     LT_MARK("k_ge_ffcount");
     size_t tb = d_temp.capacity();
@@ -482,7 +618,7 @@
     CU(cudaMemcpyAsync(h_small + o_dht, d_dht, (size_t)NS * 4 * sizeof(DhtOut), cudaMemcpyDeviceToHost, st));
     CU(cudaMemcpyAsync(h_flags + 4, d_flags, 32, cudaMemcpyDeviceToHost, st));
     CU(cudaGetLastError());
-    launches += 7;
+    launches += n;
     return true;
 }
 
@@ -511,7 +647,9 @@
     const dim3 gu1(cdiv(max_units + 1, 128), NS);
     CU(cudaMemsetAsync(d_hist, 0, (size_t)NS * 4 * 256 * 4, st));
     LT_MARK("memset");
-    k_geb_classify<<<gb, ENC_THREADS, 0, st>>>(d_comps, d_meta, d_evkey, d_tail, d_masks, d_hist);
+    CU(cudaMemsetAsync(d_corr, 0, (size_t)NS * 4, st));
+    LT_MARK("memset");
+    k_geb_classify<<<gb, ENC_THREADS, 0, st>>>(d_comps, d_meta, d_evkey, d_tail, d_masks, d_hist, d_corr);
     LT_MARK("k_geb_classify");
     size_t tb = d_temp.capacity();
     cub::DeviceScan::ExclusiveScan(d_temp, tb, d_evkey.get(), d_prev.get(), cub::Max(), -1, (int)U, st);
@@ -523,14 +661,9 @@
     LT_MARK("memset");
     k_ge_groups<<<gu1, 128, 0, st>>>(d_scans, d_meta, d_evkey, d_prev, d_tsum, d_gcount, d_hist);
     LT_MARK("k_ge_groups");
-    k_ge_tables<<<NS * 4, 32, 0, st>>>(d_hist, d_tabs, d_dht);
+    k_ge_tables<<<NS * 4, 32, 0, st>>>(d_hist, d_tabs, d_dht, d_tbits);
     LT_MARK("k_ge_tables");
-    k_geb_len<<<gb, ENC_THREADS, 0, st>>>(d_comps, d_gcount, d_tabs, d_bitlen, d_masks);
-    LT_MARK("k_geb_len");
-    tb = d_temp.capacity();
-    cub::DeviceScan::ExclusiveSum(d_temp, tb, d_bitlen.get(), d_bitoff.get(), (int)U, st);
-    LT_MARK("cub_scan");
-    launches += 7;
+    launches += 5;
     CU(cudaGetLastError());
     return true;
 }
diff --git a/caesium-clt_b200/csrc/jpeg_gpuenc.h b/caesium-clt_b200/csrc/jpeg_gpuenc.h
--- a/caesium-clt_b200/csrc/jpeg_gpuenc.h
+++ b/caesium-clt_b200/csrc/jpeg_gpuenc.h
@@ -9,7 +9,7 @@
 namespace b200 {
 
 struct DhtOut { uint8_t bits[17]; uint8_t vals[256]; int32_t nvals; };
-struct ScanOut { uint32_t total_bits, nbytes, ngroups, group_base, word_base, pad_; };
+struct ScanOut { uint32_t total_bits, nbytes, ngroups, group_base, word_base, arena_base; };
 
 class GpuEncoder {
 public:
@@ -47,7 +47,11 @@
     size_t o_scans = 0, o_total = 0, o_outlen = 0, o_dht = 0, o_comps = 0, o_flags = 0;
     DeviceBuffer<ge::Scan> d_scans;
     DeviceBuffer<BlockComp> d_comps;
-    DeviceBuffer<uint32_t> d_meta, d_tail, d_tsum, d_gcount, d_bitlen, d_bitoff;
+    DeviceBuffer<uint32_t> d_meta, d_tail, d_tsum, d_gcount;
+    DeviceBuffer<uint32_t> d_bitlen, d_bitoff;
+    DeviceBuffer<uint32_t> d_corr;
+    DeviceBuffer<unsigned long long> d_tbits;
+    DeviceBuffer<uint32_t> d_cursor, d_runlen, d_runoff, d_runpos, d_arena;
     DeviceBuffer<int> d_evkey, d_prev;
     DeviceBuffer<uint32_t> d_hist;
     DeviceBuffer<ge::Table> d_tabs;
diff --git a/caesium-clt_b200/csrc/jpeg_gpuenc_core.h b/caesium-clt_b200/csrc/jpeg_gpuenc_core.h
--- a/caesium-clt_b200/csrc/jpeg_gpuenc_core.h
+++ b/caesium-clt_b200/csrc/jpeg_gpuenc_core.h
@@ -26,6 +26,8 @@
     int rbw, rbh;
     int nblocks;
     long long unit_base;
+    long long lu_base;
+    int run_base, nruns;
     int tab_base;
     long long word_base;
     long long word_cap;
@@ -169,6 +171,11 @@
     else tail = popc64(mB & ~((2ull << last_new) - 1ull));
     return meta_pack(last_new >= 0, last_new < s.Se, tail);
 }
+template <class S>
+GE_HD int corr_bits_m(const S &s, const Masks3 &M)
+{
+    return s.mode == MODE_AC_REFINE ? popc64(mask_at(M, s.Al + 1) & band_mask(s.Ss, s.Se)) : 0;
+}
 GE_HD uint32_t classify(const Scan &s, const int16_t *blk)
 {
     if (s.mode == MODE_SEQ || s.mode == MODE_DC_FIRST) return meta_pack(true, false, 0);
@@ -185,6 +192,11 @@
 }
 
 GE_HD int eob_symbol(unsigned count) { return (nbits_of(count) - 1) << 4; }
+GE_HD int sym_extra_bits(int kind, int symbol)
+{
+    if (kind == 0) return symbol;
+    return (symbol & 15) ? (symbol & 15) : symbol == 0xF0 ? 0 : symbol >> 4;
+}
 template <class Sink>
 GE_HD void gen_eob_token(unsigned count, int tbl, Sink &sk)
 {
@@ -327,7 +339,22 @@
         if (nb > 32) { put((unsigned)(v >> 32), nb - 32); put((unsigned)v, 32); } else put((unsigned)v, nb);
     }
     GE_HD void finish() { if (n > 0) orw(wpos, cur); }
-};
+    GE_HD unsigned long long bits_written(long long word_base) const { return (unsigned long long)(wpos - word_base) * 32 + n; }
+};
+
+template <class Src, class OrFn, class StFn>
+GE_HD void place_bits(Src src, unsigned long long nbits, unsigned long long bitoff, OrFn &&orw, StFn &&stw, int k0 = 0, int dk = 1)
+{
+    if (!nbits) return;
+    const int s = (int)(bitoff & 31);
+    const long long w0 = (long long)(bitoff >> 5), nsrc = (long long)((nbits + 31) / 32), nout = (long long)((s + nbits + 31) / 32);
+    for (long long k = k0; k < nout; k += dk) {
+        const uint32_t hi = k > 0 ? src(k - 1) : 0u, lo = k < nsrc ? src(k) : 0u;
+        const uint32_t v = s ? (hi << (32 - s)) | (lo >> s) : lo;
+        if (k == 0 || k == nout - 1) { if (v) orw(w0 + k, v); }
+        else stw(w0 + k, v);
+    }
+}
 
 struct NoCount { GE_HD void operator()(uint32_t) const {} };
 template <class CountFn = NoCount>
diff --git a/caesium-clt_b200/csrc/jpeg_gpuenc_plan.h b/caesium-clt_b200/csrc/jpeg_gpuenc_plan.h
--- a/caesium-clt_b200/csrc/jpeg_gpuenc_plan.h
+++ b/caesium-clt_b200/csrc/jpeg_gpuenc_plan.h
@@ -6,6 +6,7 @@
 
 namespace b200 {
 
+constexpr int ENC_THREADS = 128;
 constexpr int ENC_MAX_VISITS = 6, ENC_AC_SLOTS = 3, ENC_DC_SLOTS = 1, ENC_DC_SYMBOLS = 17;
 constexpr int ENC_TAB_ENTRIES = ENC_AC_SLOTS * 256 + ENC_DC_SLOTS * ENC_DC_SYMBOLS;
 constexpr int ENC_DC_ENTRY = ENC_AC_SLOTS * 256;
@@ -15,6 +16,8 @@
     int mode, Ss, Se, Al, ns;
     int tbl;
     int unit_base;
+    int lu_base;
+    int run_base;
     int ac_entry;
 };
 
@@ -60,6 +63,8 @@
     int scans_per_image = 0;
     long long units_per_image = 0, words_per_image = 0;
     long long total_units = 0, total_words = 0, total_comp_blocks = 0;
+    long long total_lunits = 0;
+    int total_runs = 0, max_runs = 0;
 };
 
 inline void gpuenc_plan(const JpegGeom &g, bool progressive, const int16_t *const *coef_base, int nimages, GpuEncPlan &p)
@@ -69,7 +74,9 @@
     p.defs.assign(sc, sc + ns);
     p.scans_per_image = ns;
     p.scans.clear();
-    long long unit = 0, word = 0;
+    long long unit = 0, word = 0, lunit = 0;
+    int run = 0;
+    p.max_runs = 0;
     for (int im = 0; im < nimages; im++) {
         for (int si = 0; si < ns; si++) {
             const ScanDef &d = sc[si];
@@ -89,13 +96,16 @@
             s.rbw = g.rbw[d.ci[0]]; s.rbh = g.rbh[d.ci[0]];
             s.nblocks = d.ns > 1 ? g.mcux * g.mcuy * s.blocks_per_mcu : s.rbw * s.rbh;
             s.unit_base = unit; unit += s.nblocks;
+            s.lu_base = -1; s.run_base = -1; s.nruns = 0;
+            if (d.ns > 1) { s.lu_base = lunit; lunit += s.nblocks; }
+            else { s.run_base = run; s.nruns = (g.bw[d.ci[0]] * g.bh[d.ci[0]] + ENC_THREADS - 1) / ENC_THREADS; run += s.nruns; p.max_runs = std::max(p.max_runs, s.nruns); }
             s.tab_base = (int)p.scans.size() * 4;
             s.word_base = word; s.word_cap = (long long)s.nblocks * 32 + 64; word += s.word_cap;
             p.scans.push_back(s);
         }
         if (im == 0) { p.units_per_image = unit; p.words_per_image = word; }
     }
-    p.total_units = unit; p.total_words = word;
+    p.total_units = unit; p.total_words = word; p.total_lunits = lunit; p.total_runs = run;
     p.comps.clear(); p.max_comp_blocks = 0; p.total_comp_blocks = 0; p.on_chip = true;
     for (int im = 0; im < nimages; im++) {
         int qb = 0;
@@ -116,7 +126,7 @@
                 if (bc.nscan == ENC_MAX_VISITS || nac + ac > ENC_AC_SLOTS || ndc + dc > ENC_DC_SLOTS) { p.on_chip = false; continue; }
                 EncVisit &v = bc.visit[bc.nscan++];
                 v.scan = im * ns + si; v.mode = s.mode; v.Ss = s.Ss; v.Se = s.Se; v.Al = s.Al; v.ns = s.ns; v.tbl = s.tbl[i];
-                v.unit_base = (int)s.unit_base;
+                v.unit_base = (int)s.unit_base; v.lu_base = (int)s.lu_base; v.run_base = s.run_base;
                 v.ac_entry = ac ? nac * 256 : 0;
                 if (ac) bc.tab[nac++] = s.tab_base + 2 + v.tbl;
                 if (dc) bc.tab[ENC_AC_SLOTS + ndc++] = s.tab_base + v.tbl;
```

Measured after the change: 41890, median of 6. 1.03x the previous value.
